# jiaowoguanren0615/Segmentation_Factory

Hardware: AMD Instinct MI355X
Metric: images/sec/GPU fwd+bwd SegFormer-B0 512x512 bf16; mIoU parity vs CPU ref (higher is better)
Workload: dtype bf16; 1 GPU; SegFormer-B0 (MiT-B0 + 768-wide SegFormerHead as the reference builds it), 150 classes, 512x512, full train step (zero_grad+fwd+CE/Dice+bwd+AGC/AdamW); per_gpu_batch=256, global_batch=256, parallelism=dp1, fp8=False, inputs=resident in HBM in the captured step's input buffers (zero-copy feed), launch=hipGraph(zero_grad+fwd+loss+bwd+grad gather) + RCCL all-reduce + fused AGC/AdamW

## Files before the change

### include/segfac.h

```cpp
#ifndef SEGFAC_H
#define SEGFAC_H
#include <stdint.h>

#ifdef __cplusplus
extern "C" {
#endif

#define SEGF_F32 0
#define SEGF_BF16 1
#define SEGF_ERR_SHAPE (-1)
#define SEGF_ERR_DTYPE (-2)
#define SEGF_ERR_WORKSPACE (-3)

const char* segf_version(void);

int segf_cast(const void* src, int src_dt, void* dst, int dst_dt, int64_t n, void* stream);
int segf_cast2d(const void* src, int src_dt, int64_t ld_src, void* dst, int dst_dt, int64_t ld_dst, int64_t rows, int64_t cols,
                void* stream);
int segf_permute021(const void* in, int in_dt, void* out, int out_dt, int64_t A, int64_t Bd, int64_t Cd,
                    int64_t ld_out, void* stream);
typedef struct SegfPrepItem {
    const void* src; void* dst;
    int64_t rows, cols, ld_src, ld_dst, pb, pc;
    int32_t op, src_dt, dst_dt, reserved;
// ... 56 lines not shown
                  const float* pro_shift, int64_t rows_per_group, int act, void* stream);
int segf_bn_affine_table(const float* mean, const float* rstd, const float* gamma, const float* beta, const float* chan_scale,
                         int groups, int C, float* scale, float* shift, void* stream);
int64_t segf_gemm_dw_db_ws(int64_t M, int64_t N, int64_t K, int split_k);
int segf_gemm_dw_db(int dt, int64_t M, int64_t N, int64_t K, const void* A, int64_t lda, const void* B, int64_t ldb,
                    void* C, int c_dt, int64_t ldc, int split_k, float* ws, float* dbias, void* stream);
typedef struct SegfDwItem {
    int64_t M, N, K;
    const void* dy; int64_t lddy;
    const void* x; int64_t ldx;
    float* dw; int64_t lddw;
    float* db;
    float* ws;
    int split_k;
    int shared_split;
} SegfDwItem;
int segf_gemm_dw_db_grouped(int dt, int n, const SegfDwItem* items, void* stream);

int segf_layernorm_fwd(int dt, int64_t rows, int C, const void* x, const float* gamma, const float* beta,
                       float eps, void* y, float* mean, float* rstd, void* stream);
int64_t segf_layernorm_bwd_ws(int64_t rows, int C);
int segf_layernorm_bwd(int dt, int64_t rows, int C, const void* x, const void* dy, const float* gamma,
                       const float* mean, const float* rstd, void* dx, float* dgamma, float* dbeta,
                       float* ws, void* stream);
int segf_layernorm_bwd_fused(int dt, int64_t rows, int C, const void* x, const void* dy, const void* dy2, const void* dres,
                             const float* gamma, const float* mean, const float* rstd, void* dx, float* dgamma, float* dbeta,
                             float* ws, void* stream);
int segf_layernorm_bwd_scaled(int dt, int64_t rows, int C, const void* x, const void* dy, const void* dy2, const void* dres,
                              const float* gamma, const float* mean, const float* rstd, void* dx, float* dgamma, float* dbeta,
                              float* ws, const float* rscale, int64_t rows_per_group, void* dxs, void* stream);
int segf_layernorm_fwd_patch(int dt, int64_t rows, int C, const void* x, const float* gamma, const float* beta, float eps, void* y,
                             float* mean, float* rstd, void* y2, int log2_w, int log2_sr, void* stream);
int segf_layernorm_bwd_patch(int dt, int64_t rows, int C, const void* x, const void* dy, const void* dy2, const void* dres,
                             const float* gamma, const float* mean, const float* rstd, void* dx, float* dgamma, float* dbeta,
                             float* ws, const float* rscale, int64_t rows_per_group, void* dxs, int log2_w, int log2_sr, void* stream);
typedef struct SegfFinalizeItem { const float* partial; float* out; int64_t len; int nblk; int scatter_c; } SegfFinalizeItem;
int segf_layernorm_bwd_blocks(int64_t rows, int C);
int segf_colreduce_finalize_grouped(int n, const SegfFinalizeItem* items, void* stream);
int segf_layernorm_linear_bwd_supported(int dt, int64_t rows, int C, int N);
int segf_layernorm_linear_bwd_blocks(int64_t rows);
int64_t segf_layernorm_linear_bwd_ws(int64_t rows, int C, int N);
int segf_layernorm_linear_bwd(int dt, int64_t rows, int C, int N, const void* dh, const void* w1, const void* x, const void* y,
                              const void* dres, const float* gamma, const float* mean, const float* rstd, void* dx,
                              const float* rscale, int64_t rows_per_group, void* dxs, void* dy_out, float* dw1, float* db1,
                              float* dgamma, float* dbeta, float* ws, void* stream);
int segf_layernorm_linear_bwd_ex_supported(int dt, int64_t rows, int C, int N);
int segf_layernorm_linear_bwd_ex(int dt, int64_t rows, int C, int N, const void* dh, const void* w1, const void* x, const void* y,
                                 const float* beta, const void* dy2, int log2_w, int log2_sr, const void* dres, const float* gamma,
                                 const float* mean, const float* rstd, void* dx, const float* rscale, int64_t rows_per_group, void* dxs,
                                 void* dy_out, float* dw1, float* db1, float* dgamma, float* dbeta, float* ws, void* stream);
int segf_layernorm_linear_fwd_supported(int dt, int64_t rows, int C, int N);
int segf_layernorm_linear_fwd_blocks(int64_t rows);
int segf_layernorm_linear_fwd(int dt, int64_t rows, int C, int N, const void* x, const float* gamma, const float* beta, float eps,
                              const void* w, const float* bias, void* out, float* mean, float* rstd, void* y, void* y2, int log2_w,
                              int log2_sr, void* stream);

int64_t segf_bn_ws(int64_t rows, int C);
int segf_bn_stats(int dt, int64_t rows, int C, const void* x, float* mean, float* rstd,
                  float* running_mean, float* running_var, float momentum, float eps, float* ws, void* stream);
int segf_bn_apply(int dt, int64_t rows, int C, const void* x, const float* mean, const float* rstd,
                  const float* gamma, const float* beta, int act, const float* chan_scale,
                  int64_t rows_per_sample, void* y, void* stream);
int segf_bn_bwd(int dt, int64_t rows, int C, const void* x, const void* dy, const float* mean, const float* rstd,
                const float* gamma, const float* beta, int act, const float* chan_scale, int64_t rows_per_sample,
                int eval_mode, void* dx, float* dgamma, float* dbeta, float* ws, void* stream);

int segf_bn_cls_bwd_supported(int dt, int64_t M, int C, int K, int64_t rows_per_sample);
int64_t segf_bn_cls_bwd_ws(int64_t M, int C, int64_t rows_per_sample);
int segf_bn_cls_bwd(int dt, int64_t M, int C, int K, const void* dy, int64_t ldy, const void* w, int64_t ldw, const void* x,
                    const float* mean, const float* rstd, const float* gamma, const float* beta, int act,
                    const float* chan_scale, int64_t rows_per_sample, int eval_mode, void* dx, float* dgamma, float* dbeta,
                    float* ws, void* stream);
int segf_bn_cls_bwd_dw_supported(int dt, int64_t M, int C, int K, int64_t rows_per_sample, int C1);
int64_t segf_bn_cls_bwd_dw_ws(int64_t M, int C, int64_t rows_per_sample);
int segf_bn_cls_bwd_dw(int dt, int64_t M, int C, int K, const void* dy, int64_t ldy, const void* w, int64_t ldw, const void* x,
                       const float* mean, const float* rstd, const float* gamma, const float* beta, int act,
                       const float* chan_scale, int64_t rows_per_sample, int eval_mode, void* dx, float* dgamma,
                       float* dbeta, float* ws, const void* x1, int64_t ldx1, int C1, float* dG, void* stream);
int64_t segf_bn_cls_bwd_full_ws(int64_t M, int C, int K, int64_t rows_per_sample);
int segf_bn_cls_bwd_full(int dt, int64_t M, int C, int K, const void* dy, int64_t ldy, const void* w, int64_t ldw, const void* x,
                         const float* mean, const float* rstd, const float* gamma, const float* beta, int act,
                         const float* chan_scale, int64_t rows_per_sample, int eval_mode, void* dx, float* dgamma, float* dbeta,
                         float* ws, const void* x1, int64_t ldx1, int C1, float* dG, float* dwcls, void* stream);

int64_t segf_grn_ws(int B, int64_t rows_per_sample, int C, int bwd);
int segf_grn_fwd(int dt, int B, int64_t rows_per_sample, int C, const void* x, const float* gamma, const float* beta, void* y,
                 float* a_scratch, float* sumsq_out, float* ws, int pre_gelu, void* stream);
int segf_grn_bwd(int dt, int B, int64_t rows_per_sample, int C, const void* x, const void* dy, const float* gamma,
                 const float* sumsq_saved, void* dx, float* dgamma, float* dbeta, float* ws, int pre_gelu, void* stream);

int segf_attention_fwd(int dt, int B, int heads, int N, int Nkv, int hd, const void* q, int64_t ldq,
                       const void* k, int64_t ldk, const void* v, int64_t ldv, float scale,
                       void* o, int64_t ldo, float* lse, void* stream);
int64_t segf_attention_bwd_ws(int B, int heads, int N, int Nkv, int hd);
int segf_attention_bwd(int dt, int B, int heads, int N, int Nkv, int hd, const void* q, int64_t ldq,
                       const void* k, int64_t ldk, const void* v, int64_t ldv, float scale,
                       const void* o, int64_t ldo, const void* d_o, int64_t lddo, const float* lse,
                       void* dq, int64_t lddq, void* dk, int64_t lddk, void* dv, int64_t lddv,
                       float* ws, void* stream);

int segf_group_attention_supported(int dt, int B, int H, int W, int heads, int hd, int G, int interval, int lda);
int segf_group_attention_fwd(int dt, int B, int H, int W, int heads, int hd, int G, int interval, int lda, const void* qkv,
                             int64_t ldqkv, const float* bias, float scale, void* o, int64_t ldo, float* lse, void* stream);
int64_t segf_group_attention_bwd_ws(int B, int H, int W, int heads, int hd, int G, int interval, int lda);
int segf_group_attention_bwd(int dt, int B, int H, int W, int heads, int hd, int G, int interval, int lda, const void* qkv,
                             int64_t ldqkv, const float* bias, float scale, const void* d_o, int64_t lddo, const float* lse,
                             void* dqkv, int64_t lddqkv, float* dbias, float* ws, void* stream);

int segf_spatial_gate_supported(int dt, int B, int HW, int C, int64_t ld);
int64_t segf_spatial_gate_fwd_ws(int B, int HW, int C);
int segf_spatial_gate_fwd(int dt, int B, int HW, int C, const void* x, int64_t ldx, const void* r, const float* w, float* s, void* y,
                          int64_t ldy, float* pool, float* ws, void* stream);
int64_t segf_spatial_gate_bwd_ws(int B, int HW, int C);
int segf_spatial_gate_bwd(int dt, int B, int HW, int C, const void* dy, int64_t lddy, const float* dpool, const void* x, int64_t ldx,
                          const void* r, const float* s, const float* w, void* dx, int64_t lddx, void* dr, float* dw, float* ws,
                          void* stream);
int segf_channel_gate_mix_supported(int dt, int B, int HW, int C, int64_t ld);
int segf_channel_gate_mix_fwd(int dt, int B, int HW, int C, const void* q1, int64_t ldq, const void* k1, int64_t ldk, const float* gq,
                              const float* gk, void* u, int64_t ldu, void* stream);
int64_t segf_channel_gate_mix_bwd_ws(int B, int HW, int C);
int segf_channel_gate_mix_bwd(int dt, int B, int HW, int C, const void* du, int64_t lddu, const void* q1, int64_t ldq, const void* k1,
                              int64_t ldk, const float* gq, const float* gk, void* dq1, int64_t lddq, void* dk1, int64_t lddk, float* dgq,
                              float* dgk, float* ws, void* stream);
int segf_gated_mul_supported(int dt, int M, int C, int64_t ld);
int segf_gated_mul_fwd(int dt, int M, int C, const void* a, int64_t lda, const void* v, int64_t ldv, void* z, int64_t ldz, void* stream);
int segf_gated_mul_bwd(int dt, int M, int C, const void* dz, int64_t lddz, const void* a, int64_t lda, const void* v, int64_t ldv,
                       void* da, int64_t ldda, void* dv, int64_t lddv, void* stream);

int segf_starrelu_supported(int dt, int64_t rows, int cols, int64_t ld);
int segf_starrelu_blocks(int64_t rows, int cols);
int segf_starrelu_fwd(int dt, int64_t rows, int cols, const void* u, int64_t ldu, const float* s, const float* b, void* y, int64_t ldy,
                      void* stream);
int64_t segf_starrelu_bwd_ws(int64_t rows, int cols);
int segf_starrelu_bwd(int dt, int64_t rows, int cols, const void* u, int64_t ldu, const void* dy, int64_t lddy, const float* s, void* du,
                      int64_t lddu, float* ds, float* db, float* ws, void* stream);
int segf_colscale_supported(int dt, int64_t rows, int C, int64_t ld);
int segf_colscale_blocks(int64_t rows, int C);
int segf_colscale_fwd(int dt, int64_t rows, int C, const void* x, int64_t ldx, const float* scale, void* y, int64_t ldy, void* stream);
int64_t segf_colscale_bwd_ws(int64_t rows, int C);
int segf_colscale_bwd(int dt, int64_t rows, int C, const void* dy, int64_t lddy, const void* x, int64_t ldx, const float* scale, void* dx,
                      int64_t lddx, float* dscale, float* ws, void* stream);

int segf_dwconv3x3_gelu_fwd(int dt, int B, int H, int W, int C, const void* x, const float* w ,
                            const float* bias, int apply_gelu, void* y, void* stream);
int64_t segf_dwconv3x3_bwd_ws(int B, int H, int W, int C);
int segf_dwconv3x3_bwd_blocks(int dt, int B, int H, int W, int C);
int segf_dwconv3x3_gelu_bwd(int dt, int B, int H, int W, int C, const void* x, const float* w, const float* bias,
                            int apply_gelu, const void* dy, void* du, void* dx, float* dw, float* db,
                            float* ws, void* stream);
int segf_dwconv3x3_gelu_bwd_fc2_supported(int dt, int B, int H, int W, int C_hidden, int C_in);
int segf_dwconv3x3_gelu_bwd_fc2(int dt, int B, int H, int W, int C_hidden, int C_in, const void* f, const float* w9,
                                const float* bias, const void* dys, int64_t ld_dys, const void* w2, void* du, void* dx,
                                float* dw, float* db, float* ws, void* stream);

int segf_dwconv7x7_fwd(int dt, int B, int H, int W, int C, const void* x, const float* wt, const float* bias, void* y,
                       void* stream);
int64_t segf_dwconv7x7_bwd_ws(int B, int H, int W, int C);
int segf_dwconv7x7_bwd(int dt, int B, int H, int W, int C, const void* x, const float* wt, const void* dy, void* dx,
                       float* dw, float* db, float* ws, void* stream);

int segf_conv3x3_fwd_splitk(int mode, int B, int H, int W, int Cin, int Cout);
int segf_conv3x3_pick_splitk(int Cin, int Cout, int64_t P);
int segf_conv3x3(int mode, int B, int H, int W, int Cin, int Cout, const void* x, int64_t ldx, const void* w, int64_t ldw,
                 void* y, int y_dt, int64_t ldy, const float* bias, int split_k, float* ws, void* stream);

int segf_conv3x3_dil_live_taps(int H, int W, int dilation, int* taps );
int segf_conv3x3_dil_supported(int dt, int mode, int B, int H, int W, int Cin, int Cout, int dilation);
int segf_conv3x3_dil_pick_splitk(int B, int H, int W, int Cin, int Cout, int dilation);
int segf_conv3x3_dil(int dt, int mode, int B, int H, int W, int Cin, int Cout, int dilation, const void* x, int64_t ldx,
                     const void* w, int64_t ldw, void* y, int64_t ldy, int split_k, float* ws, void* stream);

int segf_gelu(int dt, int mode, const void* u, const void* dy, void* y, int64_t n, void* stream);
int segf_rowdot(const float* a, int64_t lda, const float* b, int64_t ldb, const float* extra_a, const float* extra_b,
                float* out, int64_t rows, int64_t cols, void* stream);
int segf_adaptive_avgpool(int dt, int bwd, int B, int H, int W, int C, int S, const void* in, void* out, void* stream);

int segf_im2col(int dt, int in_nchw_f32, int B, int H, int W, int Cin, int kh, int kw, int stride, int pad,
                int Ho, int Wo, const void* x, void* col, int64_t ldcol, void* stream);
int segf_col2im(int dt, int B, int H, int W, int Cin, int kh, int kw, int stride, int pad,
                int Ho, int Wo, const void* dcol, int64_t ldcol, void* dx, void* stream);

int segf_bilinear_fwd(int dt, int B, int h, int w, int C, const void* in, int64_t ldi,
                      int H, int W, void* out, int64_t ldo, int align_corners, void* stream);
int segf_bilinear_bwd(int dt, int B, int h, int w, int C, void* din, int64_t ldi,
                      int H, int W, const void* dout, int64_t ldo, int align_corners, void* stream);
int segf_bilinear_bwd_248(int dt, int B, int H, int W, int C, const void* dout, int64_t ldo, void* d2, void* d4, void* d8,
                          void* stream);
int segf_upsample_add(int dt, int B, int H, int W, int C, const void* base, int64_t ldb, int nsrc,
                      const void* src0, int h0, int w0, int64_t ld0, const void* src1, int h1, int w1, int64_t ld1,
                      const void* src2, int h2, int w2, int64_t ld2, void* out, int64_t ldo, int align_corners, void* stream);
int64_t segf_upsample_add_stats_ws(int B, int H, int W, int C);
int segf_upsample_add_stats(int dt, int B, int H, int W, int C, const void* base, int64_t ldb, int nsrc,
                            const void* src0, int h0, int w0, int64_t ld0, const void* src1, int h1, int w1, int64_t ld1,
                            const void* src2, int h2, int w2, int64_t ld2, void* out, int64_t ldo, int align_corners,
                            float* sums, float* ws, void* stream);
int segf_fuse_map_248_supported(int dt, int B, int H, int W, int C, int C1);
int64_t segf_fuse_map_248_ws(int B, int H, int W, int C);
int segf_fuse_map_248(int B, int H, int W, int C, int C1, const void* x1, int64_t ldx1, const void* g1, int64_t ldg,
                      const void* t2, int64_t ld2, const void* t3, int64_t ld3, const void* t4, int64_t ld4,
                      void* out, int64_t ldo, float* sums, float* ws, void* stream);
int segf_bn_stats_from_sums(const float* sums, int64_t rows, int C, float* mean, float* rstd, float* running_mean,
                            float* running_var, float momentum, float eps, void* stream);
int segf_nearest_up(int dt, int bwd, int B, int h, int w, int C, int H, int W, const void* in, const void* base, void* out,
                    void* stream);
int segf_bilinear_to_nchw_f32(int dt, int B, int h, int w, int C, const void* in, int64_t ldi,
                              int H, int W, float* out, void* stream);

int64_t segf_ce_dice_stats_floats(int B, int C);
int64_t segf_ce_dice_lse_floats(int dt, int B, int C, int h, int w, int H, int W, const void* logits, int64_t ldl);
int segf_ce_dice_fwd(int dt, int B, int C, int h, int w, int H, int W, const void* logits, int64_t ldl,
                     const int64_t* target, int64_t ignore_index, const float* class_weight, int dice,
                     float* stats, float* loss, float* pix_lse, void* stream);
int64_t segf_ce_dice_bwd_ws(int dt, int B, int C, int h, int w, int H, int W);
int segf_ce_dice_bwd(int dt, int B, int C, int h, int w, int H, int W, const void* logits, int64_t ldl,
                     const int64_t* target, int64_t ignore_index, const float* class_weight, int dice,
                     const float* stats, const float* grad_out, void* dlogits, int64_t ldd, float* ws,
                     const float* pix_lse, void* stream);

int segf_pixel_loss_supported(int dt, int mode, int B, int C, int h, int w, int H, int W);
int64_t segf_pixel_loss_state_words(int B);
int64_t segf_pixel_loss_bwd_ws(int dt, int B, int C, int h, int w, int H, int W);
int segf_pixel_loss_fwd(int dt, int mode, int B, int C, int h, int w, int H, int W, const void* logits, int64_t ldl,
                        const int64_t* target, int64_t ignore_index, const float* class_weight, float p0, float p1,
                        int size_average, float* ce_map, int32_t* state, float* loss, void* stream);
int segf_pixel_loss_bwd(int dt, int mode, int B, int C, int h, int w, int H, int W, const void* logits, int64_t ldl,
                        const int64_t* target, int64_t ignore_index, const float* class_weight, float p0, float p1,
                        int size_average, const float* ce_map, const int32_t* state, const float* grad_out, void* dlogits,
                        int64_t ldd, float* ws, void* stream);

int segf_debug_wave_reduce16(const float* in, float* out, void* stream);

int segf_argmax_confmat(int dt, int B, int C, int h, int w, int H, int W, const void* logits, int64_t ldl,
                        const int64_t* target, int64_t ignore_label, int64_t* mat, int64_t* hist,
                        int32_t* flag, int64_t* pred_out , void* stream);

#define SEGF_MSF_MAX_MAPS 16
// ... 83 lines not shown
```

### segmentation_factory_amd/csrc/conv.hip

```cpp
#include <stdlib.h>
#include "colreduce.h"

#define DW_PIX 4

template <typename T, int MODE>
__global__ void __launch_bounds__(256) dwconv3x3_kernel(const T* __restrict__ x, const float* __restrict__ w,
                                                         const float* __restrict__ bias, int apply_gelu,
                                                         const T* __restrict__ dy, T* __restrict__ y, int B, int H, int W, int C) {
    const int nchunk = C / 8;
    const int wg = (W + DW_PIX - 1) / DW_PIX;
    const int units = B * H * wg;
    const int64_t g = (int64_t)xcd_block() * 256 + threadIdx.x;
    const int ustep = (int)(((int64_t)gridDim.x * 256) / nchunk);
    const int c0 = (int)(g % nchunk) * 8;
    f32x2_t wk[9][4], bs[4];
#pragma unroll
    for (int jj = 0; jj < 4; ++jj) {
#pragma unroll
        for (int kk = 0; kk < 9; ++kk) {
            const int ks = MODE == 1 ? 8 - kk : kk;
            wk[kk][jj] = f32x2_t{w[(c0 + 2 * jj) * 9 + ks], w[(c0 + 2 * jj + 1) * 9 + ks]};
        }
        bs[jj] = (MODE != 1 && bias) ? f32x2_t{bias[c0 + 2 * jj], bias[c0 + 2 * jj + 1]} : f32x2_t{0.f, 0.f};
    }
// ... 149 lines not shown
        if (MODE == 2) { load_grow(ya - 2, grawb[0]); load_grow(ya - 1, grawb[1]); }
        int yin = ya - 1;
        for (int st = 0; st < steps; ++st) {
#pragma unroll
            for (int j = 0; j < 3; ++j, ++yin) {
                f32x2_t (&P)[DW_PIX][2] = acc[j % 3];
                f32x2_t (&Cc)[DW_PIX][2] = acc[(j + 1) % 3];
                f32x2_t (&N)[DW_PIX][2] = acc[(j + 2) % 3];
                Raw4<T> (&curc)[DW_PIX + 2] = rawb[j % 3];
                Raw4<T> (&gcurc)[DW_PIX] = grawb[j % 3];
                load_row(yin + 2, rawb[(j + 2) % 3]);
                if (MODE == 2) load_grow(yin + 1, grawb[(j + 2) % 3]);
                const bool vy = yin >= 0 && yin < H && yin <= yb;
#pragma unroll
                for (int cx = 0; cx < DW_PIX + 2; ++cx) {
                    f32x2_t v[2];
                    unpack4v(curc[cx], vy && cok[cx], v);
#pragma unroll
                    for (int kx = 0; kx < 3; ++kx) {
                        const int p = cx - kx;
                        if (p >= 0 && p < DW_PIX) {
#pragma unroll
                            for (int jj = 0; jj < 2; ++jj) {
                                P[p][jj] = wk[6 + kx][jj] * v[jj] + P[p][jj];
                                Cc[p][jj] = wk[3 + kx][jj] * v[jj] + Cc[p][jj];
                                N[p][jj] = wk[kx][jj] * v[jj] + N[p][jj];
                            }
                        }
                    }
                }
                const int yo = yin - 1;
                if (yo >= ya && yo < yb) {
                    T* orow = yo_b + (int64_t)yo * W * C;
#pragma unroll
                    for (int h = 0; h < DW_PIX / 2; ++h) {
                        f32x2_t a8[4] = {P[2 * h][0], P[2 * h][1], P[2 * h + 1][0], P[2 * h + 1][1]};
                        if (MODE == 0 && apply_gelu) gelu_erf8<false>(a8, nullptr);
                        if (MODE == 2) {
                            f32x2_t gy[4], g0[2], g1[2];
                            unpack4v(gcurc[2 * h], true, g0); unpack4v(gcurc[2 * h + 1], true, g1);
                            gy[0] = g0[0]; gy[1] = g0[1]; gy[2] = g1[0]; gy[3] = g1[1];
                            if (apply_gelu) gelu_erf8<true>(a8, gy);
                            else { a8[0] = gy[0]; a8[1] = gy[1]; a8[2] = gy[2]; a8[3] = gy[3]; }
                        }
                        const f32x2_t o0[2] = {a8[0], a8[1]}, o1[2] = {a8[2], a8[3]};
                        if (cok[2 * h + 1]) store4v(orow + coff[2 * h + 1], o0);
                        if (cok[2 * h + 2]) store4v(orow + coff[2 * h + 2], o1);
                    }
                }
#pragma unroll
                for (int p = 0; p < DW_PIX; ++p) { P[p][0] = bs[0]; P[p][1] = bs[1]; }
            }
        }
    }
}

static inline void dw_walk_plan(int H, int& R, int& nseg, int64_t columns = 0) {
    nseg = (H + 63) / 64;
    while (columns > 0 && columns * nseg < 131072 && (H + nseg - 1) / nseg > 8) nseg *= 2;
    if (POL(dw_walk_rows) > 0) nseg = (H + POL(dw_walk_rows) - 1) / POL(dw_walk_rows);
    R = (H + nseg - 1) / nseg;
}
static inline bool dw_use_walk() { return !POL(dw_no_walk); }
template <typename T, int MODE>
static inline void dw_walk_launch(hipStream_t st, const T* x, const float* w, const float* bias, int apply_gelu, const T* dy, T* y,
                                  int B, int H, int W, int C) {
    int R, nseg;
    dw_walk_plan(H, R, nseg, (int64_t)B * ((W + DW_PIX - 1) / DW_PIX) * (C / 4));
    const int64_t units = (int64_t)B * nseg * ((W + DW_PIX - 1) / DW_PIX);
    const int blocks = colfixed_blocks(units, C / 4, 1, 32768);
    hipLaunchKernelGGL((dwconv3x3_walk_kernel<T, MODE>), dim3(blocks), dim3(256), 0, st, x, w, bias, apply_gelu, dy, y, B, H, W, C, R, nseg);
}

typedef __attribute__((ext_vector_type(8))) __bf16 dwf_bf16x8;
typedef __attribute__((ext_vector_type(4))) float dwf_f32x4;
typedef __attribute__((ext_vector_type(8))) short dwf_s16x8;
typedef uint32_t dwf_u32x4 __attribute__((ext_vector_type(4)));
template <int KS>
__global__ void __launch_bounds__(256, 2) dwconv3x3_walk_fc2_kernel(const bf16_t* __restrict__ x, const float* __restrict__ w,
                                                                     const float* __restrict__ bias, const bf16_t* __restrict__ dys,
                                                                     int64_t ld_dys, const bf16_t* __restrict__ w2,
                                                                     bf16_t* __restrict__ y, int B, int H, int W, int C, int R, int nseg) {
    typedef bf16_t T;
    const int lane = threadIdx.x & 63;
    const int n = lane & 15, g = lane >> 4;
    const int nslab = C / 64;
    const int nrun = (W + 15) / 16;
    const int units = B * nseg * nrun;
    const int wv = __builtin_amdgcn_readfirstlane((int)(xcd_block() * 4 + (threadIdx.x >> 6)));
    const int ustep = (int)((gridDim.x * 4) / nslab);
    const int cbase = (wv % nslab) * 64;
    const int c0 = cbase + 4 * n;
    f32x2_t wk[9][2], bs[2];
#pragma unroll
    for (int jj = 0; jj < 2; ++jj) {
#pragma unroll
        for (int kk = 0; kk < 9; ++kk) wk[kk][jj] = f32x2_t{w[(c0 + 2 * jj) * 9 + kk], w[(c0 + 2 * jj + 1) * 9 + kk]};
        bs[jj] = bias ? f32x2_t{bias[c0 + 2 * jj], bias[c0 + 2 * jj + 1]} : f32x2_t{0.f, 0.f};
    }
    dwf_bf16x8 Bf[4][KS];
#pragma unroll
    for (int s = 0; s < KS; ++s) {
        dwf_s16x8 t[4];
#pragma unroll
        for (int e = 0; e < 8; ++e) {
            const uint2 q = *reinterpret_cast<const uint2*>(w2 + (int64_t)(32 * s + 8 * g + e) * C + c0);
            t[0][e] = (short)(q.x & 0xffffu); t[1][e] = (short)(q.x >> 16); t[2][e] = (short)(q.y & 0xffffu); t[3][e] = (short)(q.y >> 16);
        }
#pragma unroll
        for (int j = 0; j < 4; ++j) Bf[j][s] = __builtin_bit_cast(dwf_bf16x8, t[j]);
    }
    const int steps = (R + 2 + 2) / 3;
    for (int u = wv / nslab; u < units; u += ustep) {
        const int run = u % nrun;
        const int t = u / nrun;
        const int seg = t % nseg;
        const int b = t / nseg;
        const int x0 = run * 16 + 4 * g;
        const int ya = seg * R, yb = ya + R < H ? ya + R : H;
        const T* xb = x + (int64_t)b * H * W * C + c0;
        T* yo_b = y + (int64_t)b * H * W * C + c0;
        const int tpx = run * 16 + n < W ? run * 16 + n : W - 1;
        const T* gb = dys + ((int64_t)b * H * W + tpx) * ld_dys + 8 * g;
        int coff[DW_PIX + 2];
        bool cok[DW_PIX + 2];
#pragma unroll
        for (int cx = 0; cx < DW_PIX + 2; ++cx) {
            const int ix = x0 + cx - 1;
            cok[cx] = ix >= 0 && ix < W;
            coff[cx] = (ix < 0 ? 0 : (ix >= W ? W - 1 : ix)) * C;
        }
        f32x2_t acc[3][DW_PIX][2];
#pragma unroll
        for (int a = 0; a < 3; ++a)
#pragma unroll
            for (int p = 0; p < DW_PIX; ++p) { acc[a][p][0] = bs[0]; acc[a][p][1] = bs[1]; }
        Raw4<T> rawb[3][DW_PIX + 2];
        dwf_u32x4 dysb[3][KS];
        auto load_row = [&](int yin, Raw4<T> (&dst)[DW_PIX + 2]) {
            const int yc = yin < 0 ? 0 : (yin >= H ? H - 1 : yin);
            const T* row = xb + (int64_t)yc * W * C;
#pragma unroll
            for (int cx = 0; cx < DW_PIX + 2; ++cx) dst[cx] = load4_raw<T>(row + coff[cx]);
        };
        auto load_grow = [&](int yo, dwf_u32x4 (&dst)[KS]) {
            const int yc = yo < 0 ? 0 : (yo >= H ? H - 1 : yo);
            const T* row = gb + (int64_t)yc * W * ld_dys;
#pragma unroll
            for (int s = 0; s < KS; ++s) dst[s] = *reinterpret_cast<const dwf_u32x4*>(row + 32 * s);
        };
        load_row(ya - 1, rawb[0]);
        load_row(ya, rawb[1]);
        load_grow(ya - 2, dysb[0]); load_grow(ya - 1, dysb[1]);
        int yin = ya - 1;
        for (int st = 0; st < steps; ++st) {
#pragma unroll
            for (int j = 0; j < 3; ++j, ++yin) {
                f32x2_t (&P)[DW_PIX][2] = acc[j % 3];
                f32x2_t (&Cc)[DW_PIX][2] = acc[(j + 1) % 3];
                f32x2_t (&N)[DW_PIX][2] = acc[(j + 2) % 3];
                Raw4<T> (&curc)[DW_PIX + 2] = rawb[j % 3];
                dwf_u32x4 (&gcurc)[KS] = dysb[j % 3];
                load_row(yin + 2, rawb[(j + 2) % 3]);
                load_grow(yin + 1, dysb[(j + 2) % 3]);
                const bool vy = yin >= 0 && yin < H && yin <= yb;
#pragma unroll
                for (int cx = 0; cx < DW_PIX + 2; ++cx) {
                    f32x2_t v[2];
                    unpack4v(curc[cx], vy && cok[cx], v);
#pragma unroll
                    for (int kx = 0; kx < 3; ++kx) {
                        const int p = cx - kx;
                        if (p >= 0 && p < DW_PIX) {
#pragma unroll
                            for (int jj = 0; jj < 2; ++jj) {
                                P[p][jj] = wk[6 + kx][jj] * v[jj] + P[p][jj];
                                Cc[p][jj] = wk[3 + kx][jj] * v[jj] + Cc[p][jj];
                                N[p][jj] = wk[kx][jj] * v[jj] + N[p][jj];
                            }
                        }
                    }
                }
                const int yo = yin - 1;
                if (yo >= ya && yo < yb) {
                    dwf_f32x4 dgf[4];
#pragma unroll
                    for (int jm = 0; jm < 4; ++jm) {
                        dgf[jm] = dwf_f32x4{0.f, 0.f, 0.f, 0.f};
#pragma unroll
                        for (int s = 0; s < KS; ++s)
                            dgf[jm] = __builtin_amdgcn_mfma_f32_16x16x32_bf16(__builtin_bit_cast(dwf_bf16x8, gcurc[s]), Bf[jm][s], dgf[jm], 0, 0, 0);
                    }
                    T* orow = yo_b + (int64_t)yo * W * C;
#pragma unroll
                    for (int h = 0; h < DW_PIX / 2; ++h) {
                        f32x2_t a8[4] = {P[2 * h][0], P[2 * h][1], P[2 * h + 1][0], P[2 * h + 1][1]};
                        Raw4<T> q0, q1;
                        q0.u.x = pack2bf(dgf[0][2 * h], dgf[1][2 * h]); q0.u.y = pack2bf(dgf[2][2 * h], dgf[3][2 * h]);
                        q1.u.x = pack2bf(dgf[0][2 * h + 1], dgf[1][2 * h + 1]); q1.u.y = pack2bf(dgf[2][2 * h + 1], dgf[3][2 * h + 1]);
                        f32x2_t gy[4], g0[2], g1[2];
                        unpack4v(q0, true, g0); unpack4v(q1, true, g1);
                        gy[0] = g0[0]; gy[1] = g0[1]; gy[2] = g1[0]; gy[3] = g1[1];
                        gelu_erf8<true>(a8, gy);
                        const f32x2_t o0[2] = {a8[0], a8[1]}, o1[2] = {a8[2], a8[3]};
                        if (cok[2 * h + 1]) store4v(orow + coff[2 * h + 1], o0);
                        if (cok[2 * h + 2]) store4v(orow + coff[2 * h + 2], o1);
                    }
                }
#pragma unroll
                for (int p = 0; p < DW_PIX; ++p) { P[p][0] = bs[0]; P[p][1] = bs[1]; }
            }
        }
    }
}

static inline int dw_blocks(int B, int H, int W, int C) {
    return colfixed_blocks((int64_t)B * H * ((W + DW_PIX - 1) / DW_PIX), C / 8, 8, 16384);
}

extern "C" int segf_dwconv3x3_gelu_fwd(int dt, int B, int H, int W, int C, const void* x, const float* w, const float* bias,
                                       int apply_gelu, void* y, void* stream) {
    if (B <= 0 || H <= 0 || W <= 0) return 0;
    if (C <= 0 || C % 8 != 0 || ((uintptr_t)x % 16) || ((uintptr_t)y % 16)) return SEGF_ERR_SHAPE;
    if ((int64_t)B * H * W >= (1ll << 31)) return SEGF_ERR_SHAPE;
    hipStream_t st = (hipStream_t)stream;
    const int blocks = dw_blocks(B, H, W, C);
    SEGF_DISPATCH_DT(dt, T, {
        if (dw_use_walk()) dw_walk_launch<T, 0>(st, (const T*)x, w, bias, apply_gelu, (const T*)nullptr, (T*)y, B, H, W, C);
        else
        hipLaunchKernelGGL((dwconv3x3_kernel<T, 0>), dim3(blocks), dim3(256), 0, st, (const T*)x, w, bias, apply_gelu,
                           (const T*)nullptr, (T*)y, B, H, W, C);
    })
    SEGF_CHECK_LAUNCH();
    return 0;
}

#define DWG_MAX_BLOCKS 1024
struct DwgPlan { int ch, rl, slabs, nblk, units_per_blk; };
static inline DwgPlan dwg_plan(int B, int H, int W, int C) {
    DwgPlan p;
    const int nchunk = C / 8;
    p.ch = nchunk < 256 ? nchunk : 256;
    p.rl = 256 / p.ch;
    p.slabs = (nchunk + p.ch - 1) / p.ch;
    const int64_t units = (int64_t)B * H * ((W + DW_PIX - 1) / DW_PIX);
    int64_t want = cdiv64(units, (int64_t)p.rl * 4);
    int cap = DWG_MAX_BLOCKS / p.slabs;
    if (cap < 1) cap = 1;
    p.nblk = (int)(want < 1 ? 1 : (want > cap ? cap : want));
    p.units_per_blk = (int)cdiv64(units, p.nblk);
    return p;
}

template <typename T>
__global__ void __launch_bounds__(256) dwconv3x3_wgrad_kernel(const T* __restrict__ x, const T* __restrict__ du,
                                                               float* __restrict__ partial, int B, int H, int W, int C, int ch,
                                                               int rl, int units_per_blk) {
    __shared__ float red[256 * 8];
    const int tx = threadIdx.x % ch, ty = threadIdx.x / ch;
    const int chunk = blockIdx.y * ch + tx;
    const int c0 = chunk * 8;
    const bool active = ty < rl && c0 < C;
    const int wg = (W + DW_PIX - 1) / DW_PIX;
    const int units = B * H * wg;
    float acc[10][8];
#pragma unroll
    for (int o = 0; o < 10; ++o)
#pragma unroll
        for (int j = 0; j < 8; ++j) acc[o][j] = 0.f;
    (void)units_per_blk;
    if (active) {
        for (int u = (int)xcd_block() * rl + ty; u < units; u += (int)gridDim.x * rl) {
            const int xg = u % wg;
            const int t = u / wg;
// ... 316 lines not shown
static inline int dw_small_nch(int dt, int B, int H, int W, int C) {
    if (POL(dw_no_small) || C % 8 || B > 4096) return 0;
    const int HW = H * W, umax = dt == SEGF_BF16 ? 1024 : 512;
    if (HW > umax || HW < 16) return 0;
    for (int nch = 4; nch >= 1; nch >>= 1)
        if (HW * nch <= umax && (C / 8) % nch == 0) {
            if ((int64_t)B * (C / (8 * nch)) > 512 && !POL(dw_small_always)) return 0;
            return nch;
        }
    return 0;
}

extern "C" int64_t segf_dwconv3x3_bwd_ws(int B, int H, int W, int C) {
    DwgPlan p = dwg_plan(B, H, W, C > 0 ? C : 8);
    DwwPlan q = dww_plan(B, H > 0 ? H : 1, W > 0 ? W : 1, C > 0 ? C : 8);
    int nblk = p.nblk > q.nblk ? p.nblk : q.nblk;
    if (B > nblk) nblk = B;
    return (int64_t)nblk * 10 * C + 10 * (int64_t)C;
}

extern "C" int segf_dwconv3x3_gelu_bwd(int dt, int B, int H, int W, int C, const void* x, const float* w, const float* bias,
                                       int apply_gelu, const void* dy, void* du, void* dx, float* dw, float* db, float* ws,
                                       void* stream) {
    if (B <= 0 || H <= 0 || W <= 0) return 0;
    if (C <= 0 || C % 8 != 0 || ((uintptr_t)x % 16) || ((uintptr_t)dy % 16) || ((uintptr_t)du % 16) || ((uintptr_t)dx % 16))
        return SEGF_ERR_SHAPE;
    if ((int64_t)B * H * W >= (1ll << 31)) return SEGF_ERR_SHAPE;
    if (!ws) return SEGF_ERR_WORKSPACE;
    hipStream_t st = (hipStream_t)stream;
    if (const int nch = dw_small_nch(dt, B, H, W, C)) {
        const size_t esz = dt == SEGF_BF16 ? 2 : 4;
        const size_t shm = (size_t)H * W * nch * 8 * esz * 2 + (size_t)nch * 80 * 4 + 256 * 8 * 4;
        const int blocks = B * (C / (8 * nch));
        SEGF_DISPATCH_DT(dt, T, {
            hipLaunchKernelGGL((dwconv3x3_bwd_small_kernel<T>), dim3(blocks), dim3(256), shm, st, (const T*)x, w, bias, apply_gelu,
                               (const T*)dy, (T*)dx, ws, B, H, W, C, nch);
        })
        SEGF_CHECK_LAUNCH();
        if (!dw) return 0;
        float* sums_s = ws + (int64_t)B * 10 * C;
        colreduce_finalize_launch(ws, B, 10 * (int64_t)C, sums_s, st);
        SEGF_CHECK_LAUNCH();
        hipLaunchKernelGGL(dw_scatter_kernel, dim3((C + 255) / 256), dim3(256), 0, st, sums_s, C, dw, db);
        SEGF_CHECK_LAUNCH();
        return 0;
    }
    DwgPlan p = dwg_plan(B, H, W, C);
    const DwwPlan q = dww_plan(B, H, W, C);
    const bool walk = dw_use_walk();
    if (walk) p.nblk = q.nblk;
    float* sums = ws + (int64_t)p.nblk * 10 * C;
    const int blocks = dw_blocks(B, H, W, C);
    SEGF_DISPATCH_DT(dt, T, {
        if (dw_use_walk()) dw_walk_launch<T, 2>(st, (const T*)x, w, bias, apply_gelu, (const T*)dy, (T*)du, B, H, W, C);
        else
        hipLaunchKernelGGL((dwconv3x3_kernel<T, 2>), dim3(blocks), dim3(256), 0, st, (const T*)x, w, bias, apply_gelu,
                           (const T*)dy, (T*)du, B, H, W, C);
        if (walk)
        hipLaunchKernelGGL((dwconv3x3_wgrad_walk_kernel<T>), dim3(q.nblk, q.slabs), dim3(256), 0, st, (const T*)x, (const T*)du, ws,
                           B, H, W, C, q.ch, q.rl, q.R, q.nseg);
        else
        hipLaunchKernelGGL((dwconv3x3_wgrad_kernel<T>), dim3(p.nblk, p.slabs), dim3(256), 0, st, (const T*)x, (const T*)du, ws,
                           B, H, W, C, p.ch, p.rl, p.units_per_blk);
        if (dw_use_walk()) dw_walk_launch<T, 1>(st, (const T*)du, w, (const float*)nullptr, 0, (const T*)nullptr, (T*)dx, B, H, W, C);
        else
        hipLaunchKernelGGL((dwconv3x3_kernel<T, 1>), dim3(blocks), dim3(256), 0, st, (const T*)du, w, (const float*)nullptr, 0,
                           (const T*)nullptr, (T*)dx, B, H, W, C);
    })
    SEGF_CHECK_LAUNCH();
    if (!dw) return 0;
    colreduce_finalize_launch(ws, p.nblk, 10 * (int64_t)C, sums, st);
    SEGF_CHECK_LAUNCH();
    hipLaunchKernelGGL(dw_scatter_kernel, dim3((C + 255) / 256), dim3(256), 0, st, sums, C, dw, db);
    SEGF_CHECK_LAUNCH();
    return 0;
}
extern "C" int segf_dwconv3x3_bwd_blocks(int dt, int B, int H, int W, int C) {
    if (B <= 0 || H <= 0 || W <= 0 || C <= 0) return 0;
    if (dw_small_nch(dt, B, H, W, C)) return B;
    return dw_use_walk() ? dww_plan(B, H, W, C).nblk : dwg_plan(B, H, W, C).nblk;
}

#define DW_FC2_MIN_ROWS 131072
static inline bool dw_fc2_shape_ok(int dt, int B, int H, int W, int C, int Cin) {
    return dt == SEGF_BF16 && B > 0 && H > 0 && W > 0 && (Cin == 32 || Cin == 64) && C > 0 && C % 64 == 0 &&
           (int64_t)B * H * W < (1ll << 31);
}
extern "C" int segf_dwconv3x3_gelu_bwd_fc2_supported(int dt, int B, int H, int W, int C_hidden, int C_in) {
    if (!dw_fc2_shape_ok(dt, B, H, W, C_hidden, C_in)) return 0;
    if (!dw_use_walk() || dw_small_nch(dt, B, H, W, C_hidden)) return 0;
    const int pol = POL(ffn_bwd_fused);
    if (pol <= 0) return 0;
    if (pol >= 2) return 1;
    return (int64_t)B * H * W >= DW_FC2_MIN_ROWS;
}
extern "C" int segf_dwconv3x3_gelu_bwd_fc2(int dt, int B, int H, int W, int C_hidden, int C_in, const void* f, const float* w9,
                                           const float* bias, const void* dys, int64_t ld_dys, const void* w2, void* du, void* dx,
                                           float* dw, float* db, float* ws, void* stream) {
    if (B <= 0 || H <= 0 || W <= 0) return 0;
    const int C = C_hidden;
    if (dt != SEGF_BF16) return SEGF_ERR_DTYPE;
    if (!dw_fc2_shape_ok(dt, B, H, W, C, C_in) || !dw_use_walk() || dw_small_nch(dt, B, H, W, C)) return SEGF_ERR_SHAPE;
    if (((uintptr_t)f % 16) || ((uintptr_t)dys % 16) || ((uintptr_t)w2 % 16) || ((uintptr_t)du % 16) || ((uintptr_t)dx % 16) ||
        ld_dys < C_in || ld_dys % 8 != 0)
        return SEGF_ERR_SHAPE;
    if (!ws) return SEGF_ERR_WORKSPACE;
    hipStream_t st = (hipStream_t)stream;
    typedef bf16_t T;
    const DwwPlan q = dww_plan(B, H, W, C);
    float* sums = ws + (int64_t)q.nblk * 10 * C;
    {
        const int nslab = C / 64;
        const int64_t waves = (int64_t)B * q.nseg * ((W + 15) / 16) * nslab;
        int64_t blocks = (waves + 3) / 4;
        if (blocks > 32768) blocks = 32768;
        blocks = (blocks + nslab - 1) / nslab * nslab;
        if (C_in == 32)
            hipLaunchKernelGGL((dwconv3x3_walk_fc2_kernel<1>), dim3((unsigned)blocks), dim3(256), 0, st, (const T*)f, w9, bias, (const T*)dys,
                               ld_dys, (const T*)w2, (T*)du, B, H, W, C, q.R, q.nseg);
        else
            hipLaunchKernelGGL((dwconv3x3_walk_fc2_kernel<2>), dim3((unsigned)blocks), dim3(256), 0, st, (const T*)f, w9, bias, (const T*)dys,
                               ld_dys, (const T*)w2, (T*)du, B, H, W, C, q.R, q.nseg);
    }
    hipLaunchKernelGGL((dwconv3x3_wgrad_walk_kernel<T>), dim3(q.nblk, q.slabs), dim3(256), 0, st, (const T*)f, (const T*)du, ws,
                       B, H, W, C, q.ch, q.rl, q.R, q.nseg);
    dw_walk_launch<T, 1>(st, (const T*)du, w9, (const float*)nullptr, 0, (const T*)nullptr, (T*)dx, B, H, W, C);
    SEGF_CHECK_LAUNCH();
    if (!dw) return 0;
    colreduce_finalize_launch(ws, q.nblk, 10 * (int64_t)C, sums, st);
    SEGF_CHECK_LAUNCH();
    hipLaunchKernelGGL(dw_scatter_kernel, dim3((C + 255) / 256), dim3(256), 0, st, sums, C, dw, db);
    SEGF_CHECK_LAUNCH();
    return 0;
}

#define DW7_PIX 8
template <typename T, bool FLIP>
__global__ void __launch_bounds__(256) dwconv7x7_kernel(const T* __restrict__ x, const float* __restrict__ wt,
                                                         const float* __restrict__ bias, T* __restrict__ y, int B, int H, int W, int C) {
    const int nchunk = C / 8;
    const int wg = (W + DW7_PIX - 1) / DW7_PIX;
    const int units = B * H * wg;
    const int64_t g = (int64_t)xcd_block() * 256 + threadIdx.x;
    const int ustep = (int)(((int64_t)gridDim.x * 256) / nchunk);
    const int c0 = (int)(g % nchunk) * 8;
    f32x2_t bs[4];
#pragma unroll
    for (int jj = 0; jj < 4; ++jj) bs[jj] = (!FLIP && bias) ? f32x2_t{bias[c0 + 2 * jj], bias[c0 + 2 * jj + 1]} : f32x2_t{0.f, 0.f};
    for (int u = (int)(g / nchunk); u < units; u += ustep) {
        const int xg = u % wg;
        const int t = u / wg;
        const int yy = t % H;
        const int b = t / H;
        const int x0 = xg * DW7_PIX;
        f32x2_t acc[DW7_PIX][4];
#pragma unroll
        for (int p = 0; p < DW7_PIX; ++p)
#pragma unroll
            for (int jj = 0; jj < 4; ++jj) acc[p][jj] = bs[jj];
        for (int ky = 0; ky < 7; ++ky) {
            const int iy = yy + ky - 3;
            if (iy < 0 || iy >= H) continue;
            f32x2_t wk[7][4];
#pragma unroll
            for (int kx = 0; kx < 7; ++kx) {
                const float* wp = wt + (int64_t)(FLIP ? 48 - (ky * 7 + kx) : ky * 7 + kx) * C + c0;
                const float4 wa = *reinterpret_cast<const float4*>(wp), wb = *reinterpret_cast<const float4*>(wp + 4);
                wk[kx][0] = f32x2_t{wa.x, wa.y}; wk[kx][1] = f32x2_t{wa.z, wa.w};
                wk[kx][2] = f32x2_t{wb.x, wb.y}; wk[kx][3] = f32x2_t{wb.z, wb.w};
            }
            const T* row = x + (((int64_t)b * H + iy) * W) * C + c0;
#pragma unroll
            for (int half = 0; half < 2; ++half) {
                Raw8<T> raw[7];
#pragma unroll
                for (int q = 0; q < 7; ++q) {
                    const int ix = x0 + half * 7 + q - 3;
                    raw[q] = load8_raw<T>(row + (int64_t)(ix < 0 ? 0 : (ix >= W ? W - 1 : ix)) * C);
                }
                SEGF_LOADS_ISSUED();
#pragma unroll
                for (int q = 0; q < 7; ++q) {
                    const int cx = half * 7 + q;
                    const int ix = x0 + cx - 3;
                    f32x2_t v[4];
                    zero_unless(raw[q], ix >= 0 && ix < W);
                    unpack8v<T>(raw[q], v);
#pragma unroll
                    for (int kx = 0; kx < 7; ++kx) {
                        const int p = cx - kx;
                        if (p >= 0 && p < DW7_PIX) {
#pragma unroll
                            for (int jj = 0; jj < 4; ++jj) acc[p][jj] = wk[kx][jj] * v[jj] + acc[p][jj];
                        }
                    }
                }
            }
        }
#pragma unroll
        for (int p = 0; p < DW7_PIX; ++p)
// ... 450 lines not shown
```

### segmentation_factory_amd/csrc/elementwise.hip

```cpp
#include "colreduce.h"

extern "C" const char* segf_version(void) { return "segfac-hip 0.1 gfx950"; }

template <typename S, typename D>
__global__ void cast_kernel(const S* __restrict__ src, D* __restrict__ dst, int64_t n, bool vec) {
    const int64_t stride = (int64_t)gridDim.x * blockDim.x;
    if (vec) {
        const int64_t n8 = n / 8;
        for (int64_t i = (int64_t)blockIdx.x * blockDim.x + threadIdx.x; i < n8; i += stride) {
            float v[8];
            load8<S>(src + i * 8, v);
            store8<D>(dst + i * 8, v);
        }
        for (int64_t i = n8 * 8 + (int64_t)blockIdx.x * blockDim.x + threadIdx.x; i < n; i += stride)
            stf<D>(dst + i, ldf<S>(src + i));
    } else {
        for (int64_t i = (int64_t)blockIdx.x * blockDim.x + threadIdx.x; i < n; i += stride)
            stf<D>(dst + i, ldf<S>(src + i));
    }
}

extern "C" int segf_cast(const void* src, int src_dt, void* dst, int dst_dt, int64_t n, void* stream) {
    if (n <= 0) return 0;
    hipStream_t st = (hipStream_t)stream;
// ... 303 lines not shown
}
extern "C" int segf_event_destroy(void* event) { return (int)hipEventDestroy((hipEvent_t)event); }
extern "C" int segf_event_record(void* event, void* stream, int external) {
    hipStream_t st = (hipStream_t)stream;
    hipEvent_t ev = (hipEvent_t)event;
    if (!external) return (int)hipEventRecord(ev, st);
    hipStreamCaptureStatus status = hipStreamCaptureStatusNone;
    hipGraph_t graph = nullptr;
    const hipGraphNode_t* deps = nullptr;
    size_t ndeps = 0;
    hipError_t r = hipStreamGetCaptureInfo_v2(st, &status, nullptr, &graph, &deps, &ndeps);
    if (r != hipSuccess) return (int)r;
    if (status != hipStreamCaptureStatusActive) return SEGF_ERR_SHAPE;
    r = hipEventRecordWithFlags(ev, st, hipEventRecordExternal);
    if (r == hipSuccess) return 0;
    (void)hipGetLastError();
    hipGraphNode_t node = nullptr;
    r = hipGraphAddEventRecordNode(&node, graph, deps, ndeps, ev);
    if (r != hipSuccess) return (int)r;
    r = hipStreamUpdateCaptureDependencies(st, &node, 1, hipStreamSetCaptureDependencies);
    return (int)r;
}
extern "C" int segf_stream_wait_event(void* stream, void* event) {
    return (int)hipStreamWaitEvent((hipStream_t)stream, (hipEvent_t)event, 0);
}


__global__ void zero_fill_kernel(uint32_t* __restrict__ p, int64_t nwords, uint8_t* __restrict__ tail, int ntail) {
    for (int64_t i = (int64_t)blockIdx.x * blockDim.x + threadIdx.x; i < nwords; i += (int64_t)gridDim.x * blockDim.x) p[i] = 0u;
    if (blockIdx.x == 0 && (int)threadIdx.x < ntail) tail[threadIdx.x] = 0;
}
extern "C" int segf_zero(void* p, int64_t nbytes, void* stream) {
    if (nbytes <= 0) return 0;
    if ((uintptr_t)p % 4) return SEGF_ERR_SHAPE;
    const int64_t nwords = nbytes / 4;
    const int blocks = (int)imin64(cdiv64(nwords > 0 ? nwords : 1, 256), 4096);
    hipLaunchKernelGGL(zero_fill_kernel, dim3(blocks), dim3(256), 0, (hipStream_t)stream, (uint32_t*)p, nwords,
                       (uint8_t*)p + nwords * 4, (int)(nbytes - nwords * 4));
    SEGF_CHECK_LAUNCH();
    return 0;
}
__global__ void hist_accum_kernel(float* __restrict__ hist, int64_t* __restrict__ counts, int64_t n, int clear) {
    const int64_t i = (int64_t)blockIdx.x * blockDim.x + threadIdx.x;
    if (i >= n) return;
    hist[i] += (float)counts[i];
    if (clear) counts[i] = 0;
}
extern "C" int segf_hist_accum(float* hist, int64_t* counts, int64_t n, int clear, void* stream) {
    if (n <= 0) return 0;
    if (!hist || !counts) return SEGF_ERR_SHAPE;
    hipLaunchKernelGGL(hist_accum_kernel, dim3((unsigned)cdiv64(n, 256)), dim3(256), 0, (hipStream_t)stream, hist, counts, n, clear);
    SEGF_CHECK_LAUNCH();
    return 0;
}
__global__ void debug_spin_kernel(int64_t ticks) {
    const uint64_t t0 = __builtin_amdgcn_s_memrealtime();
    for (int guard = 0; guard < (1 << 24); ++guard) {
        if ((int64_t)(__builtin_amdgcn_s_memrealtime() - t0) >= ticks) break;
        __builtin_amdgcn_s_sleep(32);
    }
}
extern "C" int segf_debug_spin(int64_t us, void* stream) {
    if (us < 0 || us > 200000) return SEGF_ERR_SHAPE;
    hipLaunchKernelGGL(debug_spin_kernel, dim3(1), dim3(64), 0, (hipStream_t)stream, us * 100);
    SEGF_CHECK_LAUNCH();
    return 0;
}
__global__ void add_i64_kernel(int64_t* p, int64_t v) { if (threadIdx.x == 0) *p += v; }
extern "C" int segf_add_i64(int64_t* p, int64_t v, void* stream) {
    hipLaunchKernelGGL(add_i64_kernel, dim3(1), dim3(64), 0, (hipStream_t)stream, p, v);
    SEGF_CHECK_LAUNCH();
    return 0;
}

__device__ __forceinline__ uint64_t splitmix64(uint64_t z) {
    z += 0x9E3779B97F4A7C15ull;
    z = (z ^ (z >> 30)) * 0xBF58476D1CE4E5B9ull;
    z = (z ^ (z >> 27)) * 0x94D049BB133111EBull;
    return z ^ (z >> 31);
}
__global__ void bernoulli_scale_kernel(uint64_t* __restrict__ state, const float* __restrict__ kp, int64_t n, int64_t row_len,
                                       float* __restrict__ out) {
    const uint64_t seed = state[0], ctr = state[1];
    for (int64_t i = (int64_t)blockIdx.x * blockDim.x + threadIdx.x; i < n; i += (int64_t)gridDim.x * blockDim.x) {
        const uint64_t r = splitmix64(splitmix64(seed ^ (ctr * 0xD1B54A32D192ED03ull)) + (uint64_t)i);
        const float u = (float)(r >> 40) * (1.f / 16777216.f);
        const float k = kp[i / row_len];
        out[i] = u < k ? 1.f / k : 0.f;
    }
    __syncthreads();
    if (gridDim.x == 1 && threadIdx.x == 0) state[1] = ctr + 1;
}
extern "C" int segf_bernoulli_scale(uint64_t* state, const float* keep_prob, int64_t n, int64_t row_len, float* out, void* stream) {
    if (n <= 0) return 0;
    if (row_len <= 0 || n > (1 << 20)) return SEGF_ERR_SHAPE;
    hipLaunchKernelGGL(bernoulli_scale_kernel, dim3(1), dim3(1024), 0, (hipStream_t)stream, state, keep_prob, n, row_len, out);
    SEGF_CHECK_LAUNCH();
    return 0;
}
```

### segmentation_factory_amd/csrc/head_fused.hip

```cpp
#include "colreduce.h"

typedef __attribute__((ext_vector_type(8))) __bf16 hf_bf16x8;
typedef __attribute__((ext_vector_type(4))) float hf_f32x4;
typedef __attribute__((ext_vector_type(8))) short hf_s16x8;

struct HeadFusedArgs {
    const bf16_t* dy; int64_t ldy;
    const bf16_t* w; int64_t ldw;
    const bf16_t* x;
    const float *mean, *rstd, *gamma, *beta;
    const float* cscale;
    const float* sums;
    bf16_t* dx;
    float* partial;
    int64_t M; int C; int64_t rps; int groups_per_sample, chunks_per_sample; int act, eval_mode;
    const bf16_t* x1; int64_t ldx1;
    float* dwpart;
    float* cwpart;
};
#define DW_C1 32
#define DW_LD 40

__device__ __forceinline__ hf_bf16x8 hf_frag_tok_tr(const unsigned char* tile, int rowbytes, int cb, int lane) {
    typedef __attribute__((ext_vector_type(4))) short hf_s16x4;
    const int g = lane >> 4, i = lane & 15, q = i >> 2, p = i & 3;
    const unsigned char* a0 = tile + (8 * g + q) * rowbytes + (cb + 4 * p) * 2;
    const hf_s16x4 lo = __builtin_amdgcn_ds_read_tr16_b64_v4i16((__attribute__((address_space(3))) hf_s16x4*)a0);
    const hf_s16x4 hi = __builtin_amdgcn_ds_read_tr16_b64_v4i16((__attribute__((address_space(3))) hf_s16x4*)(a0 + 4 * rowbytes));
    const hf_s16x8 v = __builtin_shufflevector(lo, hi, 0, 1, 2, 3, 4, 5, 6, 7);
    return __builtin_bit_cast(hf_bf16x8, v);
}

__device__ __forceinline__ float hf_row_sum16(float v) {
    v += dpp_mov<DPP_XOR1>(v); v += dpp_mov<DPP_XOR2>(v); v += dpp_mov<DPP_HALF_MIRROR>(v); v += dpp_mov<DPP_MIRROR>(v);
    return v;
}

#ifndef HF_WAVES
#define HF_WAVES 8
#endif
#ifndef HF_OCC
#define HF_OCC 1
#endif
#ifndef HF_U
#define HF_U 4
#endif
template <int PASS, int KS, bool DW = false, bool CW = false>
__global__ void __launch_bounds__(64 * HF_WAVES, HF_OCC) bn_cls_bwd_kernel(HeadFusedArgs a) {
    constexpr int NT = 2;
    constexpr int TOK = 16 * HF_U;
    constexpr int RS = 32 * KS + 8;
    constexpr int NCH = TOK * 4 * KS;
    constexpr int CPT = (NCH + 64 * HF_WAVES - 1) / (64 * HF_WAVES);
    __shared__ __attribute__((aligned(16))) bf16_t tile[2][TOK][RS];
    constexpr int XW = 32 * HF_WAVES;
    constexpr int XRS = XW + 8;
    constexpr int XCH = TOK * (XW / 8);
    constexpr int XPT = XCH / (64 * HF_WAVES);
    static_assert(XCH % (64 * HF_WAVES) == 0, "x tile chunks must divide evenly over the workgroup");
    __shared__ __attribute__((aligned(16))) bf16_t xt[2][TOK][XRS];
    __shared__ __attribute__((aligned(16))) bf16_t ot[PASS == 2 ? TOK : 1][XRS];
    static_assert(!DW || (PASS == 2 && HF_WAVES == 8 && TOK == 64), "the riding weight gradient belongs to pass 2");
    static_assert(!CW || (PASS == 1 && TOK % 32 == 0), "the classifier's weight gradient rides on pass 1");
    __shared__ __attribute__((aligned(16))) bf16_t at[CW ? TOK : 1][XRS];
    hf_f32x4 accc[CW ? 2 * KS : 1][CW ? 2 : 1];
#pragma unroll
    for (int i = 0; i < (CW ? 2 * KS : 1); ++i)
#pragma unroll
        for (int j = 0; j < (CW ? 2 : 1); ++j) accc[i][j] = hf_f32x4{0.f, 0.f, 0.f, 0.f};
    constexpr int X1RS = DW_C1 + 16 + 8;
    __shared__ __attribute__((aligned(16))) bf16_t x1t[DW ? 2 : 1][DW ? TOK : 1][X1RS];
    const int lane = threadIdx.x & 63, wave = threadIdx.x >> 6;
    const int mi = lane & 15, g = lane >> 4;
    const unsigned L = xcd_block();
    const int ny = a.C / (32 * HF_WAVES);
    const int slice = (int)(L % (unsigned)ny), blk = (int)(L / (unsigned)ny);
    const int n0 = (slice * HF_WAVES + wave) * (16 * NT);
    hf_bf16x8 Wf[NT][KS];
#pragma unroll
    for (int nt = 0; nt < NT; ++nt) {
        const int n = n0 + 8 * (mi >> 2) + 4 * nt + (mi & 3);
#pragma unroll
        for (int s = 0; s < KS; ++s) {
            hf_s16x8 wv;
#pragma unroll
            for (int j = 0; j < 8; ++j) wv[j] = (short)a.w[(int64_t)(32 * s + 8 * g + j) * a.ldw + n];
            Wf[nt][s] = __builtin_bit_cast(hf_bf16x8, wv);
        }
    }
    const int f0 = n0 + 8 * g;
    float zA[8], zB[8], hC[8], hD[8], E[8], P[8], Q[8];
    const float invn = 1.f / (float)a.M;
#pragma unroll
    for (int j = 0; j < 8; ++j) {
        const float mu = a.mean[f0 + j], rs = a.rstd[f0 + j], ga = a.gamma[f0 + j], be = a.beta[f0 + j];
        zA[j] = ga * rs; zB[j] = be - mu * ga * rs;
        hC[j] = rs; hD[j] = -mu * rs;
        if (PASS == 2) {
            const float mg = a.eval_mode ? 0.f : a.sums[f0 + j] * invn, mgx = a.eval_mode ? 0.f : a.sums[a.C + f0 + j] * invn;
            E[j] = ga * rs;
            P[j] = ga * rs * (mg + hD[j] * mgx);
            Q[j] = ga * rs * hC[j] * mgx;
        }
    }
    const float zlo = a.act == 0 ? -INFINITY : 0.f, zhi = a.act == 2 ? 6.f : INFINITY;
    float s1[8], s2[8];
#pragma unroll
    for (int j = 0; j < 8; ++j) { s1[j] = 0.f; s2[j] = 0.f; }
    const int b = blk / a.chunks_per_sample, chunk = blk % a.chunks_per_sample;
    const int gbeg = (int)((int64_t)a.groups_per_sample * chunk / a.chunks_per_sample);
    const int gend = (int)((int64_t)a.groups_per_sample * (chunk + 1) / a.chunks_per_sample);
    float cs[8];
#pragma unroll
    for (int j = 0; j < 8; ++j) {
        cs[j] = a.cscale ? a.cscale[(int64_t)b * a.C + f0 + j] : 1.f;
        if (PASS == 2) E[j] *= cs[j];
        if (CW) { zA[j] *= cs[j]; zB[j] *= cs[j]; }
    }
    const int64_t row0 = (int64_t)b * a.rps;
    const int64_t last_row = row0 + (int64_t)gend * 16 - 1;
    static_assert(CPT <= 3, "dy tile: at most three 16-byte chunks per thread");
    uint4 stg0 = make_uint4(0, 0, 0, 0), stg1 = make_uint4(0, 0, 0, 0), stg2 = make_uint4(0, 0, 0, 0);
    auto fetch_one = [&](int gp, int q) -> uint4 {
        q = q < NCH ? q : NCH - 1;
        const int tk = q / (4 * KS), col = q % (4 * KS);
        int64_t m = row0 + (int64_t)gp * 16 + tk;
        m = m <= last_row ? m : last_row;
        return *reinterpret_cast<const uint4*>(a.dy + m * a.ldy + 8 * col);
    };
    auto fetch_tile = [&](int gp) {
        stg0 = fetch_one(gp, (int)threadIdx.x);
        if (CPT > 1) stg1 = fetch_one(gp, (int)threadIdx.x + 64 * HF_WAVES);
        if (CPT > 2) stg2 = fetch_one(gp, (int)threadIdx.x + 128 * HF_WAVES);
    };
    auto stash_one = [&](int bufi, int q, const uint4& v) {
        const int tk = q / (4 * KS), col = q % (4 * KS);
        if (q < NCH) *reinterpret_cast<uint4*>(&tile[bufi][tk][8 * col]) = v;
    };
    auto stash_tile = [&](int bufi) {
        stash_one(bufi, (int)threadIdx.x, stg0);
        if (CPT > 1) stash_one(bufi, (int)threadIdx.x + 64 * HF_WAVES, stg1);
        if (CPT > 2) stash_one(bufi, (int)threadIdx.x + 128 * HF_WAVES, stg2);
    };
    typedef uint32_t hf_u32x4 __attribute__((ext_vector_type(4)));
    hf_u32x4 xs[XPT];
    const int wg_f0 = slice * XW;
    auto fetch_x = [&](int gp) {
#pragma unroll
        for (int i = 0; i < XPT; ++i) {
            const int q = (int)threadIdx.x + 64 * HF_WAVES * i, tk = q / (XW / 8), c16 = q % (XW / 8);
            int64_t m = row0 + (int64_t)gp * 16 + tk;
            m = m <= last_row ? m : last_row;
            xs[i] = *reinterpret_cast<const hf_u32x4*>(a.x + m * a.C + wg_f0 + 8 * c16);
        }
    };
    auto stash_x = [&](int bufi) {
#pragma unroll
        for (int i = 0; i < XPT; ++i) {
            const int q = (int)threadIdx.x + 64 * HF_WAVES * i, tk = q / (XW / 8), c16 = q % (XW / 8);
            *reinterpret_cast<hf_u32x4*>(&xt[bufi][tk][8 * c16]) = xs[i];
        }
    };
    hf_u32x4 x1s = {0u, 0u, 0u, 0u};
    auto fetch_x1 = [&](int gp) {
        if (DW) {
            const int q = (int)threadIdx.x & 255, tk = q >> 2, c16 = q & 3;
            int64_t m = row0 + (int64_t)gp * 16 + tk;
            m = m <= last_row ? m : last_row;
            x1s = *reinterpret_cast<const hf_u32x4*>(a.x1 + m * a.ldx1 + 8 * c16);
        }
    };
    auto stash_x1 = [&](int bufi, int gp) {
        if (DW) {
            const int t = (int)threadIdx.x;
            if (t < 256) {
                const int tk = t >> 2, c16 = t & 3;
                const bool live = gp + (tk >> 4) < gend;
                const hf_u32x4 z = {0u, 0u, 0u, 0u};
                *reinterpret_cast<hf_u32x4*>(&x1t[bufi][tk][8 * c16]) = live ? x1s : z;
            } else if (t < 384) {
                const int r = t - 256, tk = r >> 1, half = r & 1;
                const bool live = gp + (tk >> 4) < gend;
                const hf_u32x4 v = {(half == 0 && live) ? 0x00003f80u : 0u, 0u, 0u, 0u};
                *reinterpret_cast<hf_u32x4*>(&x1t[bufi][tk][DW_C1 + 8 * half]) = v;
            }
        }
    };
    hf_f32x4 accw[DW ? 2 : 1][DW ? 3 : 1];
#pragma unroll
    for (int i = 0; i < (DW ? 2 : 1); ++i)
#pragma unroll
        for (int j = 0; j < (DW ? 3 : 1); ++j) accw[i][j] = hf_f32x4{0.f, 0.f, 0.f, 0.f};
    if (gbeg < gend) { fetch_tile(gbeg); fetch_x(gbeg); fetch_x1(gbeg); stash_tile(0); stash_x(0); stash_x1(0, gbeg); }
    __syncthreads();
    int bufi = 0;
    for (int gp = gbeg; gp < gend; gp += HF_U) {
        const bool more = gp + HF_U < gend;
        if (more) { fetch_tile(gp + HF_U); fetch_x(gp + HF_U); fetch_x1(gp + HF_U); }
        constexpr int UNR = CW ? 1 : HF_U;
#pragma unroll UNR
        for (int u = 0; u < HF_U; ++u) {
            hf_f32x4 acc[NT];
#pragma unroll
            for (int nt = 0; nt < NT; ++nt) acc[nt] = hf_f32x4{0.f, 0.f, 0.f, 0.f};
#pragma unroll
            for (int s = 0; s < KS; ++s) {
                const hf_bf16x8 yv = *reinterpret_cast<const hf_bf16x8*>(&tile[bufi][16 * u + mi][32 * s + 8 * g]);
#pragma unroll
                for (int nt = 0; nt < NT; ++nt) acc[nt] = __builtin_amdgcn_mfma_f32_16x16x32_bf16(Wf[nt][s], yv, acc[nt], 0, 0, 0);
            }
            const bool live = gp + u < gend;
            const hf_u32x4 xv4 = *reinterpret_cast<const hf_u32x4*>(&xt[bufi][16 * u + mi][32 * wave + 8 * g]);
            const uint32_t xw[4] = {xv4[0], xv4[1], xv4[2], xv4[3]};
            float o[8];
#pragma unroll
            for (int j = 0; j < 8; ++j) {
                const float da = j < 4 ? acc[0][j] : acc[1][j - 4];
                const float xv = (j & 1) ? __uint_as_float(xw[j >> 1] & 0xffff0000u) : __uint_as_float(xw[j >> 1] << 16);
                const float z = fmaf(xv, zA[j], zB[j]);
                const bool on = live & (z > zlo) & (z < zhi);
                const float gm = on ? da : 0.f;
                if (PASS == 1) {
                    s1[j] += gm;
                    s2[j] = fmaf(gm, xv, s2[j]);
                    if (CW) o[j] = live ? fmaxf(z, zlo) : 0.f;
                } else {
                    o[j] = fmaf(E[j], gm, -fmaf(xv, Q[j], P[j]));
                }
            }
            if (CW) {
                const hf_u32x4 av = {pack2bf(o[0], o[1]), pack2bf(o[2], o[3]), pack2bf(o[4], o[5]), pack2bf(o[6], o[7])};
                *reinterpret_cast<hf_u32x4*>(&at[16 * u + mi][32 * wave + 8 * g]) = av;
            }
            if (PASS == 2) {
                const hf_u32x4 ov = {pack2bf(o[0], o[1]), pack2bf(o[2], o[3]), pack2bf(o[4], o[5]), pack2bf(o[6], o[7])};
                *reinterpret_cast<hf_u32x4*>(&ot[16 * u + mi][32 * wave + 8 * g]) = ov;
            }
        }
        if (CW) {
            __builtin_amdgcn_fence(__ATOMIC_ACQ_REL, "wavefront");
            __builtin_amdgcn_wave_barrier();
#pragma unroll
            for (int ks = 0; ks < TOK / 32; ++ks) {
                const unsigned char* ab = reinterpret_cast<const unsigned char*>(&at[32 * ks][0]);
                const unsigned char* yb = reinterpret_cast<const unsigned char*>(&tile[bufi][32 * ks][0]);
                const hf_bf16x8 fb0 = hf_frag_tok_tr(ab, XRS * 2, 32 * wave, lane), fb1 = hf_frag_tok_tr(ab, XRS * 2, 32 * wave + 16, lane);
#pragma unroll
                for (int ct = 0; ct < 2 * KS; ++ct) {
                    const hf_bf16x8 fa = hf_frag_tok_tr(yb, RS * 2, 16 * ct, lane);
                    accc[ct][0] = __builtin_amdgcn_mfma_f32_16x16x32_bf16(fa, fb0, accc[ct][0], 0, 0, 0);
                    accc[ct][1] = __builtin_amdgcn_mfma_f32_16x16x32_bf16(fa, fb1, accc[ct][1], 0, 0, 0);
                    if (ct & 1) __builtin_amdgcn_sched_barrier(0);
                }
            }
            __builtin_amdgcn_fence(__ATOMIC_ACQ_REL, "wavefront");
            __builtin_amdgcn_wave_barrier();
        }
        __builtin_amdgcn_sched_barrier(0);
        asm volatile("" ::: "memory");
        if (more) {
            stash_tile(bufi ^ 1);
            stash_x(bufi ^ 1);
            stash_x1(bufi ^ 1, gp + HF_U);
        }
        __syncthreads();
        if (DW) {
#pragma unroll
            for (int ks = 0; ks < TOK / 32; ++ks) {
                const unsigned char* ob = reinterpret_cast<const unsigned char*>(&ot[32 * ks][0]);
                const unsigned char* xb = reinterpret_cast<const unsigned char*>(&x1t[bufi][32 * ks][0]);
                const hf_bf16x8 fa0 = hf_frag_tok_tr(ob, XRS * 2, 32 * wave, lane), fa1 = hf_frag_tok_tr(ob, XRS * 2, 32 * wave + 16, lane);
#pragma unroll
                for (int nt = 0; nt < 3; ++nt) {
                    const hf_bf16x8 fb = hf_frag_tok_tr(xb, X1RS * 2, 16 * nt, lane);
                    accw[0][nt] = __builtin_amdgcn_mfma_f32_16x16x32_bf16(fa0, fb, accw[0][nt], 0, 0, 0);
                    accw[1][nt] = __builtin_amdgcn_mfma_f32_16x16x32_bf16(fa1, fb, accw[1][nt], 0, 0, 0);
                }
            }
        }
        if (PASS == 2) {
#pragma unroll
            for (int i = 0; i < XPT; ++i) {
                const int q = (int)threadIdx.x + 64 * HF_WAVES * i, tk = q / (XW / 8), c16 = q % (XW / 8);
                const hf_u32x4 ov = *reinterpret_cast<const hf_u32x4*>(&ot[tk][8 * c16]);
                if (gp + (tk >> 4) < gend)
                    *reinterpret_cast<hf_u32x4*>(a.dx + (row0 + (int64_t)gp * 16 + tk) * a.C + wg_f0 + 8 * c16) = ov;
            }
            __syncthreads();
        }
        bufi ^= 1;
    }
    if (DW) {
        float* dst = a.dwpart + ((int64_t)blk * a.C + wg_f0 + 32 * wave) * DW_LD;
#pragma unroll
        for (int mt = 0; mt < 2; ++mt)
#pragma unroll
            for (int nt = 0; nt < 3; ++nt) {
                const int cc = 16 * nt + mi;
                if (cc < DW_LD) {
#pragma unroll
                    for (int r = 0; r < 4; ++r) dst[(16 * mt + 4 * g + r) * DW_LD + cc] = accw[mt][nt][r];
                }
            }
    }
    if (CW) {
        float* dst = a.cwpart + (int64_t)blk * (32 * KS) * a.C + wg_f0 + 32 * wave + mi;
#pragma unroll
        for (int ct = 0; ct < 2 * KS; ++ct)
#pragma unroll
            for (int ft = 0; ft < 2; ++ft)
#pragma unroll
                for (int r = 0; r < 4; ++r) dst[(int64_t)(16 * ct + 4 * g + r) * a.C + 16 * ft] = accc[ct][ft][r];
    }
    if (PASS == 1) {
        float* dst = a.partial + (int64_t)blk * 2 * a.C + f0;
#pragma unroll
        for (int j = 0; j < 8; ++j) {
            const float r1 = hf_row_sum16(s1[j]), r2 = hf_row_sum16(s2[j]);
            const float csj = a.cscale ? a.cscale[(int64_t)b * a.C + f0 + j] : 1.f;
            const float hCj = a.rstd[f0 + j], hDj = -a.mean[f0 + j] * hCj;
            if (mi == 0) { dst[j] = csj * r1; dst[a.C + j] = csj * fmaf(hCj, r2, hDj * r1); }
        }
    }
}

__global__ void hf_split_kernel(const float* __restrict__ sums, int C, float* __restrict__ dgamma, float* __restrict__ dbeta) {
    const int c = blockIdx.x * blockDim.x + threadIdx.x;
    if (c >= C) return;
    dbeta[c] = sums[c];
    dgamma[c] = sums[C + c];
}

static int hf_chunks(int B, int groups_per_sample, int ny, bool cw = false) {
    const int budget = cw ? 768 : 3072;
    int s = (budget / ny + B - 1) / B;
    if (s > groups_per_sample / 8) s = groups_per_sample / 8;
    return s < 1 ? 1 : s;
}

extern "C" int segf_bn_cls_bwd_supported(int dt, int64_t M, int C, int K, int64_t rows_per_sample) {
    if (dt != SEGF_BF16 || POL(no_head_fused)) return 0;
    if (K % 32 || K < 32 || K > 192 || C % (32 * HF_WAVES) || rows_per_sample <= 0 || rows_per_sample % 16 || M % rows_per_sample) return 0;
    if (M / rows_per_sample > 65535 || M < 16384) return 0;
    return 1;
}
extern "C" int64_t segf_bn_cls_bwd_ws(int64_t M, int C, int64_t rows_per_sample) {
    const int B = (int)(M / rows_per_sample);
    return (int64_t)B * hf_chunks(B, (int)(rows_per_sample / 16), C / (32 * HF_WAVES)) * 2 * C + 2 * C;
}

extern "C" int64_t segf_bn_cls_bwd_full_ws(int64_t M, int C, int K, int64_t rows_per_sample) {
    const int B = (int)(M / rows_per_sample);
    const int gps = (int)(rows_per_sample / 16), ny = C / (32 * HF_WAVES);
    const int64_t nb_cw = (int64_t)B * hf_chunks(B, gps, ny, true), nb_plain = (int64_t)B * hf_chunks(B, gps, ny, false);
    const int64_t nblk = nb_cw > nb_plain ? nb_cw : nb_plain;
    return nblk * 2 * C + 2 * C + nblk * C * DW_LD + nb_cw * (int64_t)K * C;
}

extern "C" int segf_bn_cls_bwd_dw_supported(int dt, int64_t M, int C, int K, int64_t rows_per_sample, int C1) {
    if (POL(no_head_fused_dw)) return 0;
    return segf_bn_cls_bwd_supported(dt, M, C, K, rows_per_sample) && C1 == DW_C1 && K <= 160;
}
extern "C" int64_t segf_bn_cls_bwd_dw_ws(int64_t M, int C, int64_t rows_per_sample) {
    const int B = (int)(M / rows_per_sample);
    return segf_bn_cls_bwd_ws(M, C, rows_per_sample) +
           (int64_t)B * hf_chunks(B, (int)(rows_per_sample / 16), C / (32 * HF_WAVES)) * C * DW_LD;
}

static int bn_cls_bwd_impl(int dt, int64_t M, int C, int K, const void* dy, int64_t ldy, const void* w, int64_t ldw, const void* x,
                           const float* mean, const float* rstd, const float* gamma, const float* beta, int act,
                           const float* chan_scale, int64_t rows_per_sample, int eval_mode, void* dx, float* dgamma,
                           float* dbeta, float* ws, const void* x1, int64_t ldx1, float* dG, void* stream, float* dwcls = nullptr);

extern "C" int segf_bn_cls_bwd_full(int dt, int64_t M, int C, int K, const void* dy, int64_t ldy, const void* w, int64_t ldw,
                                    const void* x, const float* mean, const float* rstd, const float* gamma, const float* beta, int act,
                                    const float* chan_scale, int64_t rows_per_sample, int eval_mode, void* dx, float* dgamma,
                                    float* dbeta, float* ws, const void* x1, int64_t ldx1, int C1, float* dG, float* dwcls,
                                    void* stream) {
    if (x1 && (!segf_bn_cls_bwd_dw_supported(dt, M, C, K, rows_per_sample, C1) || !dG || ldx1 < C1 || ldx1 % 8 || ((uintptr_t)x1 % 16)))
        return SEGF_ERR_SHAPE;
    if (dwcls && (K > 192 || act > 1)) return SEGF_ERR_SHAPE;
    return bn_cls_bwd_impl(dt, M, C, K, dy, ldy, w, ldw, x, mean, rstd, gamma, beta, act, chan_scale, rows_per_sample, eval_mode, dx,
                           dgamma, dbeta, ws, x1, ldx1, x1 ? dG : nullptr, stream, dwcls);
}

extern "C" int segf_bn_cls_bwd(int dt, int64_t M, int C, int K, const void* dy, int64_t ldy, const void* w, int64_t ldw, const void* x,
                               const float* mean, const float* rstd, const float* gamma, const float* beta, int act,
                               const float* chan_scale, int64_t rows_per_sample, int eval_mode, void* dx, float* dgamma,
                               float* dbeta, float* ws, void* stream) {
    return bn_cls_bwd_impl(dt, M, C, K, dy, ldy, w, ldw, x, mean, rstd, gamma, beta, act, chan_scale, rows_per_sample, eval_mode, dx,
                           dgamma, dbeta, ws, nullptr, 0, nullptr, stream);
}
extern "C" int segf_bn_cls_bwd_dw(int dt, int64_t M, int C, int K, const void* dy, int64_t ldy, const void* w, int64_t ldw, const void* x,
                                  const float* mean, const float* rstd, const float* gamma, const float* beta, int act,
                                  const float* chan_scale, int64_t rows_per_sample, int eval_mode, void* dx, float* dgamma,
                                  float* dbeta, float* ws, const void* x1, int64_t ldx1, int C1, float* dG, void* stream) {
    if (!segf_bn_cls_bwd_dw_supported(dt, M, C, K, rows_per_sample, C1) || !x1 || !dG || ldx1 < C1 || ldx1 % 8 || ((uintptr_t)x1 % 16))
        return SEGF_ERR_SHAPE;
    return bn_cls_bwd_impl(dt, M, C, K, dy, ldy, w, ldw, x, mean, rstd, gamma, beta, act, chan_scale, rows_per_sample, eval_mode, dx,
                           dgamma, dbeta, ws, x1, ldx1, dG, stream);
}

static int bn_cls_bwd_impl(int dt, int64_t M, int C, int K, const void* dy, int64_t ldy, const void* w, int64_t ldw, const void* x,
                           const float* mean, const float* rstd, const float* gamma, const float* beta, int act,
                           const float* chan_scale, int64_t rows_per_sample, int eval_mode, void* dx, float* dgamma,
                           float* dbeta, float* ws, const void* x1, int64_t ldx1, float* dG, void* stream, float* dwcls) {
    if (!segf_bn_cls_bwd_supported(dt, M, C, K, rows_per_sample) || ldy < K || ldw < C || act < 0 || act > 2) return SEGF_ERR_SHAPE;
    if (((uintptr_t)dy | (uintptr_t)x | (uintptr_t)dx) % 16 || (ldy % 8)) return SEGF_ERR_SHAPE;
    if (!ws) return SEGF_ERR_WORKSPACE;
    hipStream_t st = (hipStream_t)stream;
    const int B = (int)(M / rows_per_sample), gps = (int)(rows_per_sample / 16), ny = C / (32 * HF_WAVES);
    const int chunks = hf_chunks(B, gps, ny, dwcls != nullptr);
    const int nblk = B * chunks;
    float* sums = ws + (int64_t)nblk * 2 * C;
    float* dwpart = sums + 2 * C;
    float* cwpart = dwpart + (int64_t)nblk * C * DW_LD;
    HeadFusedArgs a{(const bf16_t*)dy, ldy, (const bf16_t*)w, ldw, (const bf16_t*)x, mean, rstd, gamma, beta, chan_scale, sums,
                    (bf16_t*)dx, ws, M, C, rows_per_sample, gps, chunks, act, eval_mode, (const bf16_t*)x1, ldx1, dwpart, cwpart};
    const dim3 grid((unsigned)(nblk * ny));
#define HF_LAUNCH(PASS)                                                                                                  \
    do {                                                                                                                 \
        switch (K / 32) {                                                                                                \
        case 1: hipLaunchKernelGGL((bn_cls_bwd_kernel<PASS, 1>), grid, dim3(64 * HF_WAVES), 0, st, a); break;                      \
        case 2: hipLaunchKernelGGL((bn_cls_bwd_kernel<PASS, 2>), grid, dim3(64 * HF_WAVES), 0, st, a); break;                      \
        case 3: hipLaunchKernelGGL((bn_cls_bwd_kernel<PASS, 3>), grid, dim3(64 * HF_WAVES), 0, st, a); break;                      \
        case 4: hipLaunchKernelGGL((bn_cls_bwd_kernel<PASS, 4>), grid, dim3(64 * HF_WAVES), 0, st, a); break;                      \
        case 5: hipLaunchKernelGGL((bn_cls_bwd_kernel<PASS, 5>), grid, dim3(64 * HF_WAVES), 0, st, a); break;                      \
        default: hipLaunchKernelGGL((bn_cls_bwd_kernel<PASS, 6>), grid, dim3(64 * HF_WAVES), 0, st, a); break;                     \
        }                                                                                                                \
    } while (0)
    if (dwcls) {
        switch (K / 32) {
        case 1: hipLaunchKernelGGL((bn_cls_bwd_kernel<1, 1, false, true>), grid, dim3(64 * HF_WAVES), 0, st, a); break;
        case 2: hipLaunchKernelGGL((bn_cls_bwd_kernel<1, 2, false, true>), grid, dim3(64 * HF_WAVES), 0, st, a); break;
        case 3: hipLaunchKernelGGL((bn_cls_bwd_kernel<1, 3, false, true>), grid, dim3(64 * HF_WAVES), 0, st, a); break;
        case 4: hipLaunchKernelGGL((bn_cls_bwd_kernel<1, 4, false, true>), grid, dim3(64 * HF_WAVES), 0, st, a); break;
        case 5: hipLaunchKernelGGL((bn_cls_bwd_kernel<1, 5, false, true>), grid, dim3(64 * HF_WAVES), 0, st, a); break;
        default: hipLaunchKernelGGL((bn_cls_bwd_kernel<1, 6, false, true>), grid, dim3(64 * HF_WAVES), 0, st, a); break;
        }
        SEGF_CHECK_LAUNCH();
        colreduce_finalize_launch(cwpart, nblk, (int64_t)K * C, dwcls, st);
    } else {
        HF_LAUNCH(1);
    }
    SEGF_CHECK_LAUNCH();
    colreduce_finalize_launch(ws, nblk, 2 * (int64_t)C, sums, st);
    SEGF_CHECK_LAUNCH();
    if (x1) {
        switch (K / 32) {
        case 1: hipLaunchKernelGGL((bn_cls_bwd_kernel<2, 1, true>), grid, dim3(64 * HF_WAVES), 0, st, a); break;
        case 2: hipLaunchKernelGGL((bn_cls_bwd_kernel<2, 2, true>), grid, dim3(64 * HF_WAVES), 0, st, a); break;
        case 3: hipLaunchKernelGGL((bn_cls_bwd_kernel<2, 3, true>), grid, dim3(64 * HF_WAVES), 0, st, a); break;
        case 4: hipLaunchKernelGGL((bn_cls_bwd_kernel<2, 4, true>), grid, dim3(64 * HF_WAVES), 0, st, a); break;
        default: hipLaunchKernelGGL((bn_cls_bwd_kernel<2, 5, true>), grid, dim3(64 * HF_WAVES), 0, st, a); break;
        }
        SEGF_CHECK_LAUNCH();
        colreduce_finalize_launch(dwpart, nblk, (int64_t)C * DW_LD, dG, st);
    } else {
        HF_LAUNCH(2);
    }
    SEGF_CHECK_LAUNCH();
#undef HF_LAUNCH
    hipLaunchKernelGGL(hf_split_kernel, dim3((C + 255) / 256), dim3(256), 0, st, sums, C, dgamma, dbeta);
    SEGF_CHECK_LAUNCH();
    return 0;
}
```

### segmentation_factory_amd/csrc/loss.hip

```cpp
#include <stdlib.h>
#include "colreduce.h"

#include "loss_geom.h"

static inline int pow2_scale(int h, int w, int H, int W) {
    if (h <= 0 || w <= 0 || H % h || W % w) return 0;
    const int sc = H / h;
    if (W / w != sc || (sc & (sc - 1)) || sc > 8) return 0;
    return sc;
}

template <typename T, int NS>
__device__ __forceinline__ void load_tap(const T* __restrict__ p, int lane, int C, float (&t)[NS]) {
#pragma unroll
    for (int s = 0; s < NS; ++s) {
        const int c = lane + 64 * s;
        const float v = ldf<T>(p + (c < C ? c : C - 1));
        t[s] = c < C ? v : 0.f;
    }
}

template <typename T, int NS, bool ATEN = false>
__device__ __forceinline__ void pixel_logits(const T* __restrict__ img, const LossGeom& g, int Y, int X, int lane, float (&z)[NS]) {
    if (g.h == g.H && g.w == g.W) {
// ... 288 lines not shown
#pragma unroll
    for (int s = 0; s < NS; ++s) { aI[s] = 0.f; aP[s] = 0.f; aT[s] = 0.f; }
    float ce = 0.f, wsum = 0.f, nvalid = 0.f, bad = 0.f;
    for (int cell = blockIdx.x * 4 + wave; cell < ncell; cell += gridDim.x * 4) {
        const Cell c = make_cell(cell / ncx - halo, cell % ncx - halo, g.h, g.w, halo);
        float t00[NS], t01[NS], t10[NS], t11[NS];
        load_cell_taps<T, NS>(img, g, c, lane, t00, t01, t10, t11);
        const int codes = cell_label_codes(tg, g, sc, off, c.cj, c.ck, lane, ignore_index);
        const float mb = cell_max_bound<NS>(t00, t01, t10, t11, lane, g.C);
        for (int a = 0; a < sc; ++a) {
            const int Y = sc * c.cj + off + a;
            if (Y < 0 || Y >= g.H) continue;
            const float ly = (a + 0.5f) * inv_sc * fhalo;
            float L[NS], R[NS];
#pragma unroll
            for (int s = 0; s < NS; ++s) {
                L[s] = (1.f - ly) * t00[s] + ly * t10[s];
                R[s] = (1.f - ly) * t01[s] + ly * t11[s];
            }
            for (int bb = 0; bb < sc; ++bb) {
                const int t = __builtin_amdgcn_readlane(codes, a * sc + bb);
                if (t == -1) continue;
                if (t == -2) { bad = 1.f; continue; }
                const float lx = (bb + 0.5f) * inv_sc * fhalo;
                float z[NS], pr[NS];
#pragma unroll
                for (int s = 0; s < NS; ++s) z[s] = (lane + 64 * s) < g.C ? (1.f - lx) * L[s] + lx * R[s] : -INFINITY;
                const float lse = wave_softmax_bounded<NS>(z, mb, pr);
                const float wt = cw ? cw[t] : 1.f;
                nvalid += 1.f; wsum += wt;
#pragma unroll
                for (int s = 0; s < NS; ++s) {
                    aP[s] += pr[s];
                    if (lane + 64 * s == t) { aI[s] += pr[s]; aT[s] += 1.f; ce += wt * (lse - z[s]); }
                }
            }
        }
    }
    ce = wave_sum_all(ce);
    fwd_block_tail<NS>(aI, aP, aT, ce, wsum, nvalid, bad, lane, wave, g.C,
                       partial + ((int64_t)blockIdx.x * g.B + b) * (3 * g.C + 4));
}

template <typename T, int NS>
__global__ void __launch_bounds__(LS_THREADS) ce_dice_fwd_kernel(const T* __restrict__ logits, LossGeom g,
                                                                  const int64_t* __restrict__ target, int64_t ignore_index,
                                                                  const float* __restrict__ cw, float* __restrict__ partial) {
    const int lane = threadIdx.x & 63;
    const int wave = __builtin_amdgcn_readfirstlane(threadIdx.x >> 6);
    const int b = blockIdx.y;
    const int64_t npix = (int64_t)g.H * g.W;
    const int64_t nw = (int64_t)gridDim.x * 4;
    const int64_t per = (npix + nw - 1) / nw;
    const int64_t wid = (int64_t)blockIdx.x * 4 + wave;
    const int64_t p0 = wid * per, p1 = p0 + per < npix ? p0 + per : npix;
    const T* img = logits + (int64_t)b * g.h * g.w * g.ldl;
    const int64_t* tg = target + (int64_t)b * npix;
    float aI[NS], aP[NS], aT[NS];
#pragma unroll
    for (int s = 0; s < NS; ++s) { aI[s] = 0.f; aP[s] = 0.f; aT[s] = 0.f; }
    float ce = 0.f, wsum = 0.f, nvalid = 0.f, bad = 0.f;
    for (int64_t p = p0; p < p1; ++p) {
        const int64_t t = tg[p];
        if (t == ignore_index) continue;
        if (t < 0 || t >= g.C) { bad = 1.f; continue; }
        const int Y = (int)(p / g.W), X = (int)(p - (int64_t)Y * g.W);
        float z[NS], pr[NS];
        pixel_logits<T, NS>(img, g, Y, X, lane, z);
        const float lse = wave_softmax<NS>(z, pr);
        const float wt = cw ? cw[t] : 1.f;
        nvalid += 1.f; wsum += wt;
#pragma unroll
        for (int s = 0; s < NS; ++s) {
            aP[s] += pr[s];
            if (lane + 64 * s == (int)t) { aI[s] += pr[s]; aT[s] += 1.f; ce += wt * (lse - z[s]); }
        }
    }
    ce = wave_sum_all(ce);
    fwd_block_tail<NS>(aI, aP, aT, ce, wsum, nvalid, bad, lane, wave, g.C,
                       partial + ((int64_t)blockIdx.x * g.B + b) * (3 * g.C + 4));
}

__global__ void __launch_bounds__(256) ce_dice_loss_kernel(float* __restrict__ stats, int B, int C, int dice, float* __restrict__ loss) {
    __shared__ float red[256];
    __shared__ float tail[4];
    const int stride = 3 * C + 4;
    float dsum = 0.f;
    for (int i = threadIdx.x; i < B * C; i += 256) {
        const int b = i / C, c = i - b * C;
        const float* st = stats + (int64_t)b * stride;
        const float I = st[c], P = st[C + c], T = st[2 * C + c];
        float sets = P + T;
        if (sets == 0.f) sets = 2.f * I;
        dsum += (2.f * I + LS_EPS) / (sets + LS_EPS);
    }
    red[threadIdx.x] = dsum;
    if (threadIdx.x < 4) {
        float s = 0.f;
        for (int b = 0; b < B; ++b) s += stats[(int64_t)b * stride + 3 * C + threadIdx.x];
        tail[threadIdx.x] = s;
    }
    __syncthreads();
    for (int o = 128; o > 0; o >>= 1) {
        if (threadIdx.x < o) red[threadIdx.x] += red[threadIdx.x + o];
        __syncthreads();
    }
    if (threadIdx.x == 0) {
        float* st = stats + (int64_t)B * stride;
        st[0] = tail[0]; st[1] = tail[1]; st[2] = tail[2]; st[3] = tail[3];
        const float ce = tail[0] / tail[1];
        const float dl = dice ? 1.f - red[0] / (float)(B * C) : 0.f;
        loss[0] = ce + dl; loss[1] = ce; loss[2] = dl;
    }
}

template <int NS>
__device__ __forceinline__ void dice_coefs(const float* __restrict__ stats, int b, int B, int C, int dice, int lane,
                                           float (&gI)[NS], float (&gP)[NS]) {
    const float* st = stats + (int64_t)b * (3 * C + 4);
#pragma unroll
    for (int s = 0; s < NS; ++s) {
        const int c = lane + 64 * s;
        float a = 0.f, bb = 0.f;
        if (c < C && dice) {
            const float I = st[c], P = st[C + c], Tt = st[2 * C + c];
            const float sets = P + Tt;
            if (sets != 0.f) {
                const float nbc = 1.f / (float)(B * C);
                a = -nbc * 2.f / (sets + LS_EPS);
                bb = nbc * (2.f * I + LS_EPS) / ((sets + LS_EPS) * (sets + LS_EPS));
            }
        }
        gI[s] = a; gP[s] = bb;
    }
}
template <int NS>
__device__ __forceinline__ void pixel_grad(const float (&z)[NS], int t, int lane, const float (&gI)[NS], const float (&gP)[NS],
                                           float wce, float go, float (&dz)[NS], float mb = INFINITY) {
    float pr[NS], G[NS];
    if (mb == INFINITY) wave_softmax<NS>(z, pr); else wave_softmax_bounded<NS>(z, mb, pr);
    float dot = 0.f;
#pragma unroll
    for (int s = 0; s < NS; ++s) {
        G[s] = gP[s] + (lane + 64 * s == t ? gI[s] : 0.f);
        dot += G[s] * pr[s];
    }
    dot = wave_sum_all(dot);
#pragma unroll
    for (int s = 0; s < NS; ++s)
        dz[s] = go * (pr[s] * (G[s] - dot) + wce * (pr[s] - (lane + 64 * s == t ? 1.f : 0.f)));
}

template <typename T, int NS>
__global__ void __launch_bounds__(LS_THREADS) ce_dice_bwd_cells_kernel(const T* __restrict__ logits, LossGeom g, int sc,
                                                                        const int64_t* __restrict__ target, int64_t ignore_index,
                                                                        const float* __restrict__ cw, int dice,
                                                                        const float* __restrict__ stats,
                                                                        const float* __restrict__ grad_out, T* __restrict__ dlow,
                                                                        int64_t ldd, const int* __restrict__ run_if) {
    if (run_if && __hip_atomic_load(run_if, __ATOMIC_RELAXED, __HIP_MEMORY_SCOPE_AGENT) == 0) return;
    __shared__ float accum[LS_TILE * LS_TILE][64 * NS];
    const int lane = threadIdx.x & 63;
    const int wave = __builtin_amdgcn_readfirstlane(threadIdx.x >> 6);
    const int b = blockIdx.y;
    const int tiles_x = (g.w + LS_TILE - 1) / LS_TILE;
    const int ty0 = (blockIdx.x / tiles_x) * LS_TILE, tx0 = (blockIdx.x % tiles_x) * LS_TILE;
    const int halo = sc > 1 ? 1 : 0, off = sc >> 1;
    const float inv_sc = 1.f / (float)sc, fhalo = (float)halo;
    for (int i = threadIdx.x; i < LS_TILE * LS_TILE * 64 * NS; i += LS_THREADS) (&accum[0][0])[i] = 0.f;
    float gI[NS], gP[NS];
    dice_coefs<NS>(stats, b, g.B, g.C, dice, lane, gI, gP);
    const float go = grad_out ? grad_out[0] : 1.f;
    const float invW = 1.f / stats[(int64_t)g.B * (3 * g.C + 4) + 1];
    const T* img = logits + (int64_t)b * g.h * g.w * g.ldl;
    const int64_t* tg = target + (int64_t)b * g.H * g.W;
    __syncthreads();
    const int ncl = LS_TILE + halo;
    const int ncol = halo ? 4 : 1;
    for (int col = 0; col < ncol; ++col) {
        const int pj = col >> 1, pk = col & 1;
        const int nj = halo ? (ncl - pj + 1) / 2 : ncl, nk = halo ? (ncl - pk + 1) / 2 : ncl;
        for (int idx = wave; idx < nj * nk; idx += 4) {
            const int lj = halo ? 2 * (idx / nk) + pj : idx / nk, lk = halo ? 2 * (idx % nk) + pk : idx % nk;
            const int cj = ty0 - halo + lj, ck = tx0 - halo + lk;
// ... 1003 lines not shown
```

### segmentation_factory_amd/csrc/policy.h

```cpp
#pragma once

#define SEGF_POLICY_TABLE(X)                                                                                                             \
                                                                                                   \
    X(gemm_no_big, "SEGFAC_GEMM_NO_BIG", 0, "never take the 256 x 256-tile kernel (gemm_bf16_big_kernel): everything on the 128-tile one") \
    X(gemm_no_skinny, "SEGFAC_GEMM_NO_SKINNY", 0, "no streaming products for K, N <= 128 (gemm_skinny_kernel and its relatives)")        \
    X(gemm_no_skinny_rows, "SEGFAC_GEMM_NO_SKINNY_ROWS", 0, "the [tokens x 32] -> 768 projection on gemm_skinny_kernel instead of the whole-row form") \
    X(gemm_no_skinny_k, "SEGFAC_GEMM_NO_SKINNY_K", 0, "no K-split streaming product for 32- / 64-wide outputs (gemm_skinny_k_kernel)")  \
    X(gemm_no_dw_skinny, "SEGFAC_GEMM_NO_DW_SKINNY", 0, "small-output weight gradients on the tiled split-K kernel instead of gemm_dw_skinny_kernel") \
    X(gemm_no_narrow, "SEGFAC_GEMM_NO_NARROW", 0, "256-tile kernel: full 128 x 64 wave tiles also for outputs <= 160 wide (bit-identical results)") \
    X(gemm_no_deep, "SEGFAC_GEMM_NO_DEEP", 0, "256-tile forward: one K step of operand loads in flight instead of two")                  \
    X(gemm_no_deep128, "SEGFAC_GEMM_NO_DEEP128", 0, "128-tile kernel: one K step in flight instead of two")                              \
    X(gemm_no_fastload, "SEGFAC_GEMM_NO_FASTLOAD", 0, "guarded tile loads everywhere (no workgroup-uniform guard-free full-K-step loads)") \
    X(gemm_no_tr, "SEGFAC_GEMM_NO_TR", 0, "debugging: reduction-major fragments by scalar LDS reads instead of ds_read_b64_tr_b16; disables every kernel built on the transposed read") \
    X(gemm_no_pro, "SEGFAC_GEMM_NO_PRO", 0, "segf_gemm_pro_supported answers 0: BatchNorm + ReLU + Dropout2d are applied by their own pass") \
    X(gemm_no_fused_db, "SEGFAC_GEMM_NO_FUSED_DB", 0, "bias gradient as its own column-sum launch instead of riding on the weight-gradient product") \
    X(no_grouped_dw, "SEGFAC_NO_GROUPED_DW", 0, "segf_gemm_dw_db_grouped runs its members one by one")                                   \
    X(dw_no_xcd_slabs, "SEGFAC_DW_NO_XCD_SLABS", 0, "split-K weight gradients (128-tile kernel) in hardware workgroup order instead of one K slab per XCD")                \
    X(dw_no_shared_split, "SEGFAC_DW_NO_SHARED_SPLIT", 0, "grouped weight gradients keep their per-layer slice counts (also read by the host layer)") \
    X(no_wide_reduce, "SEGFAC_NO_WIDE_REDUCE", 0, "split-K partials of large outputs summed by the 16 x 16 form instead of whole rows")   \
    X(no_reduce4, "SEGFAC_NO_REDUCE4", 0, "split-K reduce: one output per thread instead of four (bitwise the same sums)")               \
    X(gemm_f32_no_mfma, "SEGFAC_GEMM_F32_NO_MFMA", 0, "fp32 storage (exact-parity mode, evaluate): products on the vector FMA kernel instead of the f32 matrix instruction") \
    X(gemm8_linear, "SEGFAC_GEMM8_LINEAR", 1, "0: plain nn.Linear products never take the eight-phase kernel (the 256 / 128 tile kernels as in r04)") \
    X(gemm8_linear_min_tiles, "SEGFAC_GEMM8_LINEAR_MIN_TILES", 128, "fewest 256 x 256 tiles for which a K >= 2048 nn.Linear product takes the eight-phase kernel (192 for shorter K)") \
    X(gemm8_linear_min_fill, "SEGFAC_GEMM8_LINEAR_MIN_FILL", 60, "smallest share (percent) of the launched 256 x 256 tiles that must be output for an nn.Linear product with ragged last tiles to take the eight-phase kernel") \
    X(gemm8_linear_min_k, "SEGFAC_GEMM8_LINEAR_MIN_K", 256, "shortest reduction for which an nn.Linear product takes the eight-phase kernel (its 12-load prologue and drain against K / 64 tiles)") \
    X(gemm8_dw, "SEGFAC_GEMM8_DW", 1, "0: nn.Linear weight gradients never take the eight-phase kernel below 65536 tokens (the grouped 128-tile kernel as in r04)") \
    X(gemm8_dw_min_gflop, "SEGFAC_GEMM8_DW_MIN_GFLOP", 100, "smallest nn.Linear weight gradient (GFLOP; both feature counts multiples of 256, >= 256 FLOP per operand byte) that takes the eight-phase kernel + a column-sum pass instead of the grouped 128-tile kernel") \
    X(gemm8_linear_min_gflop, "SEGFAC_GEMM8_LINEAR_MIN_GFLOP", 36, "smallest nn.Linear product (GFLOP, K >= 512; 100 for shorter K) that takes the eight-phase kernel") \
                                 \
    X(no_gemm8, "SEGFAC_NO_GEMM8", 0, "no eight-phase kernel at all (gemm8_kernel): the two-phase 256-tile kernel everywhere")           \
    X(no_gemm8t, "SEGFAC_NO_GEMM8T", 0, "no eight-phase kernel for weight gradients (reduction-major operands)")                         \
    X(conv_no_fwd_split, "SEGFAC_CONV_NO_FWD_SPLIT", 0, "3 x 3 forward / data gradient with few output tiles: no split over the (channel block, tap) walk") \
    X(g8_stagger, "SEGFAC_G8_STAGGER", -1, "eight-phase kernel: 1 = wave groups one barrier apart, 0 = lockstep, -1 = staggered for bf16 and the per-device choice (segf_gemm8_option) for fp8") \
    X(no_fp8, "SEGFAC_NO_FP8", 0, "segf_gemm_fp8_supported answers 0 (block-scaled 128-tile fp8 GEMM)")                                  \
    X(no_fp8_conv, "SEGFAC_NO_FP8_CONV", 0, "segf_conv3x3_fp8*_supported answer 0")                                                      \
    X(no_fp8_wgrad, "SEGFAC_NO_FP8_WGRAD", 0, "fp8 3 x 3 convolutions keep a bf16 weight gradient")                                      \
    X(no_fp8_linear, "SEGFAC_NO_FP8_LINEAR", 0, "segf_linear_fp8_supported answers 0")                                                   \
                                                                             \
    X(dilconv_no_cull, "SEGFAC_DILCONV_NO_CULL", 0, "dilated 3 x 3 convolution: all nine taps are walked, with zero loads where a tap leaves the image, instead of the live taps only") \
                                                                            \
    X(attn_no_mfma, "SEGFAC_ATTN_NO_MFMA", 0, "attention on the VALU reference kernels (attention.hip) also in bf16")                    \
    X(attn_f32_no_mfma, "SEGFAC_ATTN_F32_NO_MFMA", 0, "fp32 attention forward on the vector kernel (one query per lane) instead of the f32 matrix instruction") \
    X(attn64_prescale, "SEGFAC_ATTN64_PRESCALE", 0, "head dim 64, >= 128 keys: scale log2(e) rides on the Q fragments (bf16(q c), one more rounding per q element) and -max / -lse are the score accumulators' initial values, instead of one multiply-add per score: forward + query-side backward, +8 % / +2 % per kernel, attention error x 1.2 - 2.3") \
    X(attn64_dkv_rows, "SEGFAC_ATTN64_DKV_ROWS", 128, "head dim 64, >= 128 keys, key-side backward: query rows per staged Q / dO tile and barrier (128, 64 or 32: the same arithmetic, bit for bit)") \
    X(attn_no_fused_bwd, "SEGFAC_ATTN_NO_FUSED_BWD", 0, "head dim 32, <= 256 keys: query-side + key-side backward kernels instead of the one-kernel backward") \
    X(attn32_classic, "SEGFAC_ATTN32_CLASSIC", 0, "head dim 32 backward (one-kernel and key-side kernels): the round-2 score arithmetic (subtract, multiply, __expf; (dP - D) scale per score) instead of P = exp2(S c - lse log2(e)) with -D as the C operand of the dP products and the scale applied once to dK and dQ") \
                                                                                \
    X(dw_no_walk, "SEGFAC_DW_NO_WALK", 0, "depthwise 3 x 3: the round-1 strip kernels instead of the vertical-walk kernels")             \
    X(dw_walk_rows, "SEGFAC_DW_WALK_ROWS", 0, "depthwise 3 x 3 walk: rows per segment (0 = chosen from the map size)")                   \
    X(dw_no_small, "SEGFAC_DW_NO_SMALL", 0, "depthwise 3 x 3 backward of small maps: three passes instead of the one-launch LDS form")   \
    X(dw_small_always, "SEGFAC_DW_SMALL_ALWAYS", 0, "... the one-launch form beyond one round of workgroups as well")                    \
    X(ffn_bwd_fused, "SEGFAC_FFN_BWD_FUSED", 1, "Mix-FFN backward, fc2's data gradient formed inside pass A of the depthwise backward (segf_dwconv3x3_gelu_bwd_fc2_supported): 0 = never, 1 = from 131072 token rows on, 2 = wherever the shape has the kernel") \
                                                           \
    X(no_fuse_map, "SEGFAC_NO_FUSE_MAP", 0, "folded SegFormerHead map: streaming product + VALU upsample-add instead of fuse_map_kernel") \
    X(no_bwd248_mfma, "SEGFAC_NO_BWD248_MFMA", 0, "transposed 1/2-1/4-1/8 resizes on the VALU kernel instead of fuse_map_bwd_kernel")    \
    X(upadd_generic, "SEGFAC_UPADD_GENERIC", 0, "upsample-add: the generic per-source kernels also for the 2-4-8 pyramid")               \
    X(no_head_fused, "SEGFAC_NO_HEAD_FUSED", 0, "segf_bn_cls_bwd_supported answers 0: classifier data gradient and BatchNorm backward as separate passes") \
    X(no_head_fused_dw, "SEGFAC_NO_HEAD_FUSED_DW", 0, "the folded head's stage-1 weight gradient does not ride on pass 2 of the fused BatchNorm backward") \
                                                                                 \
    X(loss_no_band, "SEGFAC_LOSS_NO_BAND", 0, "CE / Dice forward and backward on the tile kernels instead of the band sweep")            \
    X(loss_no_band_fwd, "SEGFAC_LOSS_NO_BAND_FWD", 0, "... the forward only")                                                             \
    X(loss_band_rows, "SEGFAC_LOSS_BAND_ROWS", 0, "band sweep: rows per segment (0 = 16)")                                               \
    X(loss_no_mfma, "SEGFAC_LOSS_NO_MFMA", 0, "ratio-4 loss kernels on the VALU cells form (fp32 storage)")                              \
    X(loss_no_retry, "SEGFAC_LOSS_NO_RETRY", 0, "no exact per-pixel retry pass behind the flagged cells")                                \
    X(loss_no_lse, "SEGFAC_LOSS_NO_LSE", 0, "the backward recomputes the softmax normalisation instead of taking the forward's per-pixel log-sum") \
                                                                                                     \
    X(ln_linear_bwd_fused, "SEGFAC_LN_LINEAR_BWD_FUSED", 1, "Mix-FFN backward, fc1's data / weight / bias gradients formed inside the LayerNorm backward of norm2 (segf_layernorm_linear_bwd_supported): 0 = never, 1 = from 131072 token rows on, 2 = wherever the shape has the kernel") \
    X(ln_linear_fwd_fused, "SEGFAC_LN_LINEAR_FWD_FUSED", 1, "MiT stages 1 / 2: LayerNorm as the operand prologue of its thin Linear (norm2 -> fc1, norm1 -> q; segf_layernorm_linear_fwd_supported), the LayerNorm output neither stored nor saved, and norm1 -> q's backward in one pass where SEGFAC_LN_LINEAR_BWD_FUSED allows it too: 0 = never, 1 = from 131072 token rows on, 2 = wherever the shape has the kernel") \
                                                                                                 \
    X(no_wide_finalize, "SEGFAC_NO_WIDE_FINALIZE", 0, "column-reduction finalize: one output per thread instead of four (bitwise the same sums)") \
                                                                                 \
    X(no_ln_patch, "SEGFAC_NO_LN_PATCH", 0, "[host] MiT blocks: im2col / col2im around the spatial-reduction conv instead of the patch-major LayerNorm output") \
    X(no_scaled_ln_bwd, "SEGFAC_NO_SCALED_LN_BWD", 0, "[host] DropPath backward as its own scale_rows launch instead of riding on the LayerNorm backward") \
    X(no_deferred_dw, "SEGFAC_NO_DEFERRED_DW", 0, "[host] weight gradients issued layer by layer inside the captured step (no grouped launches)") \
    X(no_deferred_finalize, "SEGFAC_NO_DEFERRED_FINALIZE", 0, "[host] LayerNorm dgamma / dbeta finalizes issued one by one")              \
    X(no_head_fused_cw, "SEGFAC_NO_HEAD_FUSED_CW", 0, "[host] the classifier's weight gradient as its own product instead of riding on pass 1 of the fused BatchNorm backward") \
    X(no_bwd248, "SEGFAC_NO_BWD248", 0, "[host] folded head backward: three segf_bilinear_bwd launches instead of the one-pass segf_bilinear_bwd_248") \
    X(no_gelu_grn, "SEGFAC_NO_GELU_GRN", 0, "[host] ConvNeXtV2 blocks: GELU as its own pass in front of the GRN kernels")                \
    X(no_weight_shadow, "SEGFAC_NO_WEIGHT_SHADOW", 0, "[host] captured step: weights cast to bf16 per use instead of one cast of the flat buffer") \
    X(no_derived_weights, "SEGFAC_NO_DERIVED_WEIGHTS", 0, "[host] captured step: derived weight layouts built in front of each layer instead of one grouped launch")

struct SegfPolicy {
#define SEGF_POLICY_FIELD(field, env, def, doc) int field;
    SEGF_POLICY_TABLE(SEGF_POLICY_FIELD)
#undef SEGF_POLICY_FIELD
    int g8_stagger_fp8;
};

const SegfPolicy& segf_policy();
#define POL(field) (segf_policy().field)

struct SegfTrace {
    int on;
    int dry;
    int n;
    const char* names[256];
    const char* where[256];
};
SegfTrace& segf_trace();
void segf_trace_note(const char* kernel_text, const char* where);
```

### segmentation_factory_amd/functional.py

```python
import contextlib

import torch
from torch.autograd import Function

from . import hip


def _rowmajor(t):
    return t if t.stride(-1) == 1 else t.contiguous()


_SHADOW = None


class shadow_scope:
    def __init__(self, table):
        self.table = table

    def __enter__(self):
        global _SHADOW
        self.prev, _SHADOW = _SHADOW, self.table
        return self

    def __exit__(self, *exc):
# ... 1034 lines not shown
    @staticmethod
    def backward(ctx, dy):
        x, sc = ctx.saved_tensors
        gs = gslot(ctx, 1)
        dx, dscale = hip.colscale_bwd(_rowmajor(dy), x, sc, dscale=gs.view(-1) if gs is not None and gs.is_contiguous() else None)
        return dx, dscale.view(ctx.pshape)


def col_scale(x, scale):
    return ColScaleFn.apply(x, scale)


@direct_grads(1, 2)
class DWConvGeluFn(Function):

    @staticmethod
    def forward(ctx, x, weight, bias, B, H, W, apply_gelu):
        x = x if x.is_contiguous() else x.contiguous()
        Cc = x.shape[1]
        w9 = weight.detach().reshape(Cc, 9).contiguous()
        b = bias.detach().contiguous() if bias is not None else None
        y = hip.dwconv3x3_gelu_fwd(x, w9, b, B, H, W, Cc, apply_gelu)
        ctx.save_for_backward(x, w9, b)
        ctx.meta = (B, H, W, Cc, apply_gelu, weight.shape)
        return y

    @staticmethod
    def backward(ctx, dy):
        x, w9, b = ctx.saved_tensors
        B, H, W, Cc, apply_gelu, wshape = ctx.meta
        dy = dy if dy.is_contiguous() else dy.contiguous()
        gw, gb = gslot(ctx, 1), (gslot(ctx, 2) if b is not None else None)
        if _FIN_QUEUE is not None and _adjacent_slots(ctx, 1, 2) is not None:
            dx, item = hip.dwconv3x3_gelu_bwd(x, w9, b, dy, B, H, W, Cc, apply_gelu, dw_out=gw, db_out=gb, defer=True)
            _queue_finalizes(ctx, (item, (1, 2)))
            return dx, None, None, None, None, None, None
        dx, dw, db = hip.dwconv3x3_gelu_bwd(x, w9, b, dy, B, H, W, Cc, apply_gelu, dw_out=gw, db_out=gb)
        return dx, dw.view(wshape), (db if b is not None else None), None, None, None, None


def dwconv3x3_gelu(x, weight, bias, B, H, W, apply_gelu=True):
    return DWConvGeluFn.apply(x, weight, bias, B, H, W, apply_gelu)


@direct_grads(1, 2, 3, 4)
class DWConvGeluLinearFn(Function):

    @staticmethod
    def forward(ctx, x, weight2, bias2, weight, bias, B, H, W, residual, rscale):
        x = x if x.is_contiguous() else x.contiguous()
        M, Cc = x.shape
        N = weight2.shape[0]
        w9 = weight.detach().reshape(Cc, 9).contiguous()
        b = bias.detach().contiguous()
        g = hip.dwconv3x3_gelu_fwd(x, w9, b, B, H, W, Cc, True)
        w2 = _w(weight2.reshape(N, -1), x.dtype)
        y = hip.gemm(0, g, w2, M, N, Cc, bias=bias2.detach(), residual=residual, rscale=rscale, rows_per_group=H * W)
        ctx.save_for_backward(x, w9, b, g, w2, rscale)
        ctx.meta = (B, H, W, Cc, N, M, weight.shape, weight2.shape, residual is not None)
        return y

    @staticmethod
    def backward(ctx, dy):
        x, w9, b, g, w2, rscale = ctx.saved_tensors
        B, H, W, Cc, N, M, wshape, w2shape, has_res = ctx.meta
        dy = _rowmajor(dy)
        dys = _scaled_dy(dy, rscale, H * W) if rscale is not None else dy
        dw2, db2 = _linear_param_grads(ctx, dys, g, N, Cc, M, 1, 2, True, w2shape)
        gw, gb = gslot(ctx, 3), gslot(ctx, 4)
        dres = dy if (has_res and ctx.needs_input_grad[8]) else None
        if _FIN_QUEUE is not None and _adjacent_slots(ctx, 3, 4) is not None:
            dx, item = hip.dwconv3x3_gelu_bwd_fc2(x, w9, b, dys, w2, B, H, W, Cc, N, dw_out=gw, db_out=gb, defer=True)
            _queue_finalizes(ctx, (item, (3, 4)))
            return dx, dw2, db2, None, None, None, None, None, dres, None
        dx, dw, db = hip.dwconv3x3_gelu_bwd_fc2(x, w9, b, dys, w2, B, H, W, Cc, N, dw_out=gw, db_out=gb)
        return dx, dw2, db2, dw.view(wshape), db, None, None, None, dres, None


def dwconv3x3_gelu_linear_ok(x, weight2, bias2, weight, bias, B, H, W):
    if not (x.is_cuda and x.dtype == torch.bfloat16 and torch.is_grad_enabled() and x.requires_grad):
        return False
    if bias is None or bias2 is None or not all(p.requires_grad for p in (weight2, bias2, weight, bias)):
        return False
    return hip.dwconv3x3_gelu_bwd_fc2_supported(x.dtype, B, H, W, x.shape[1], weight2.shape[0])


def dwconv3x3_gelu_linear(x, weight2, bias2, weight, bias, B, H, W, residual=None, rscale=None):
    y = DWConvGeluLinearFn.apply(x, weight2, bias2, weight, bias, B, H, W, residual, rscale)
    if rscale is not None:
        y._segf_dp = (rscale, H * W)
    return y


def _bn_mean_rstd(x, training, pre_sums, running_mean, running_var, momentum, eps):
    if training and pre_sums is not None:
        return hip.bn_stats_from_sums(pre_sums, x.shape[0], running_mean, running_var, momentum, eps)
    if training:
        return hip.bn_stats(x, running_mean, running_var, momentum, eps)
    return running_mean.detach().clone(), torch.rsqrt(running_var.detach() + eps)


@direct_grads(1, 2)
class BatchNormActFn(Function):

    @staticmethod
    def forward(ctx, x, gamma, beta, running_mean, running_var, training, momentum, eps, act, chan_scale, rows_per_sample,
                pre_sums=None):
        x = x if x.is_contiguous() else x.contiguous()
        g, b = gamma.detach().contiguous(), beta.detach().contiguous()
        mean, rstd = _bn_mean_rstd(x, training, pre_sums, running_mean, running_var, momentum, eps)
        y = hip.bn_apply(x, mean, rstd, g, b, act, chan_scale, rows_per_sample or 1)
        ctx.save_for_backward(x, mean, rstd, g, b, chan_scale)
        ctx.meta = (act, rows_per_sample or 1, not training)
        return y

    @staticmethod
    def backward(ctx, dy):
        x, mean, rstd, g, b, chan_scale = ctx.saved_tensors
        act, rps, eval_mode = ctx.meta
        dy = dy if dy.is_contiguous() else dy.contiguous()
        dx, dg, db = hip.bn_bwd(x, dy, mean, rstd, g, b, act, chan_scale, rps, eval_mode)
        return dx, dg, db, None, None, None, None, None, None, None, None, None


def batch_norm_act(x, gamma, beta, running_mean, running_var, training, momentum=0.1, eps=1e-5, act=1, chan_scale=None,
                   rows_per_sample=None, pre_sums=None):
    return BatchNormActFn.apply(x, gamma, beta, running_mean, running_var, training, momentum, eps, act, chan_scale,
                                rows_per_sample, pre_sums)


@direct_grads(1, 2, 11, 12)
class BnActLinearFn(Function):

    @staticmethod
    def forward(ctx, x, gamma, beta, running_mean, running_var, training, momentum, eps, act, chan_scale, rps, weight, bias, Np,
                pre_sums, fold_slot=None):
        ctx.fold_slot = fold_slot
        x = x if x.is_contiguous() else x.contiguous()
        M, K = x.shape
        N = weight.shape[0]
        g, b = gamma.detach().contiguous(), beta.detach().contiguous()
        mean, rstd = _bn_mean_rstd(x, training, pre_sums, running_mean, running_var, momentum, eps)
        scale, shift = hip.bn_affine_table(mean, rstd, g, b, chan_scale, M // rps, K)
        w, bp = _padded_rows(weight, bias, N, Np, K, x.dtype, x.device)
        y = hip.gemm_pro(0, x, w, M, Np, K, scale, shift, rps, act, bias=bp)[:, :N]
        ctx.save_for_backward(x, mean, rstd, g, b, chan_scale, scale, shift, w)
        ctx.meta = (M, N, K, Np, act, rps, not training, bias is not None, weight.shape)
        return y

    @staticmethod
    def backward(ctx, dy):
        x, mean, rstd, g, b, chan_scale, scale, shift, w = ctx.saved_tensors
        M, N, K, Np, act, rps, eval_mode, has_bias, wshape = ctx.meta
        if dy.stride(-1) == 1 and dy.stride(0) == Np:
            dyp = dy.as_strided((M, Np), (Np, 1))
        else:
            dyp = hip.zeros((M, Np), x.dtype, x.device)
            hip.cast2d(_rowmajor(dy), dyp[:, :N])
        db = hip.colsum(dyp)[:N] if has_bias else None
        dw = None
        if hip.bn_cls_bwd_supported(x.dtype, M, K, Np, rps):
            slot = ctx.fold_slot
            x1 = slot.get('x1') if slot is not None else None
            ride_dg = x1 is not None and x1.shape[0] == M and hip.bn_cls_bwd_dw_supported(x.dtype, M, K, Np, rps, x1.shape[1])
            if act in (0, 1) and not hip.policy('no_head_fused_cw'):
                dx, dg, dbeta, dG, dwc = hip.bn_cls_bwd_full(dyp, w, x, mean, rstd, g, b, act, chan_scale, rps, eval_mode,
                                                             x1=x1 if ride_dg else None)
                dw = dwc[:N].view(wshape)
                if ride_dg:
                    slot['dG'] = dG
            elif ride_dg:
                dx, dg, dbeta, slot['dG'] = hip.bn_cls_bwd_dw(dyp, w, x, mean, rstd, g, b, act, chan_scale, rps, eval_mode, x1)
            else:
                dx, dg, dbeta = hip.bn_cls_bwd(dyp, w, x, mean, rstd, g, b, act, chan_scale, rps, eval_mode)
        else:
            da = hip.gemm(1, dyp, w, M, K, Np)
            dx, dg, dbeta = hip.bn_bwd(x, da, mean, rstd, g, b, act, chan_scale, rps, eval_mode)
        if dw is None:
            dw = hip.gemm_pro(2, dyp, x, Np, K, M, scale, shift, rps, act, split_k=_splitk(Np, K, M))[:N].view(wshape)
        return dx, dg, dbeta, None, None, None, None, None, None, None, None, dw, db, None, None, None


def bn_act_linear(x, gamma, beta, running_mean, running_var, training, momentum, eps, act, chan_scale, rows_per_sample, weight,
                  bias, pad_to=None, pre_sums=None):
    M, K = x.shape
    N = weight.shape[0]
    Np = pad_to if (pad_to and pad_to > N) else N
    rps = rows_per_sample or M
    if (x.dtype == torch.bfloat16 and act in (0, 1) and M % rps == 0 and hip.gemm_pro_supported(x.dtype, 0, M, Np, K, rps)
            and hip.gemm_pro_supported(x.dtype, 2, Np, K, M, rps)):
        return BnActLinearFn.apply(x, gamma, beta, running_mean, running_var, training, momentum, eps, act, chan_scale, rps,
                                   weight, bias, Np, pre_sums, getattr(x, '_segf_fold', None))
    y = batch_norm_act(x, gamma, beta, running_mean, running_var, training, momentum, eps, act, chan_scale, rows_per_sample,
                       pre_sums=pre_sums)
    return linear(y, weight, bias, pad_to=pad_to)


@direct_grads(5, 6, 7, 8, 9, 10, 11, 12)
class SegformerProjectConcatFn(Function):

    @staticmethod
    def forward(ctx, geoms, *args):
        feats, weights, biases = args[0:4], args[4:8], args[8:12]
        B = geoms[0][0]
        H1, W1 = geoms[0][1], geoms[0][2]
        E = weights[0].shape[0]
        dtype = feats[0].dtype
        M1 = B * H1 * W1
        cat = torch.empty((M1, 4 * E), dtype=dtype, device=feats[0].device)
        saved = []
        for i in range(4):
            f = _rowmajor(feats[i])
            w = _w(weights[i], dtype)
            _, h, wd = geoms[i]
            sl = cat[:, (3 - i) * E:(4 - i) * E]
            if i == 0:
                hip.gemm(0, f, w, M1, E, f.shape[1], out=sl, bias=biases[i].detach())
            else:
                t = hip.gemm(0, f, w, B * h * wd, E, f.shape[1], bias=biases[i].detach())
                hip.bilinear_fwd(t, B, h, wd, E, H1, W1, sl, align_corners=False)
            saved += [f, w]
        ctx.save_for_backward(*saved)
        ctx.meta = (geoms, E)
        return cat

    @staticmethod
    def backward(ctx, dcat):
        geoms, E = ctx.meta
        saved = ctx.saved_tensors
        dcat = _rowmajor(dcat)
        B, H1, W1 = geoms[0]
        dfs, dws, dbs = [], [], []
        for i in range(4):
            f, w = saved[2 * i], saved[2 * i + 1]
            _, h, wd = geoms[i]
            sl = dcat[:, (3 - i) * E:(4 - i) * E]
            dy = sl if i == 0 else hip.bilinear_bwd(sl, B, h, wd, E, H1, W1, align_corners=False)
            M, Ci = f.shape
            dfs.append(hip.gemm(1, dy, w, M, Ci, E) if ctx.needs_input_grad[1 + i] else None)
            dws.append(hip.gemm(2, dy, f, E, Ci, M, out_dtype=torch.float32, split_k=_splitk(E, Ci, M)))
            dbs.append(hip.colsum(dy))
        return (None, *dfs, *dws, *dbs)


def segformer_project_concat(feats, weights, biases, geoms):
    return SegformerProjectConcatFn.apply(tuple(geoms), *feats, *weights, *biases)


@direct_grads(5, 6, 7, 8, 9, 10, 11, 12, 13)
class SegformerFoldedFuseFn(Function):
# ... 624 lines not shown
```

### segmentation_factory_amd/hip.py

```python
import ctypes as C
import math
import os
import re

import torch

_HERE = os.path.dirname(os.path.abspath(__file__))
LIB_PATH = os.environ.get('SEGFAC_HIP_LIB') or os.path.join(_HERE, 'libsegfac_hip.so')
HEADER_PATH = os.path.normpath(os.path.join(_HERE, '..', 'include', 'segfac.h'))
F32, BF16 = 0, 1
ERR_SHAPE = -1
_lib = None

_i, _l, _f, _p = C.c_int, C.c_int64, C.c_float, C.c_void_p
_SCALAR = {'int': _i, 'int32_t': _i, 'int64_t': _l, 'float': _f}
_POINTEE = {'void', 'char', 'int', 'int32_t', 'int64_t', 'uint8_t', 'uint64_t', 'float'}


def _ctype(ctype, where, structs):
    t = re.sub(r'\bconst\b', ' ', ctype).replace('*', ' * ').split()
    if t and all(w == '*' for w in t[1:]):
        base, stars = t[0], len(t) - 1
        if stars == 0 and base in _SCALAR:
            return _SCALAR[base]
# ... 771 lines not shown
    y = torch.empty_like(x)
    _chk(lib().segf_bn_apply(dt_of(x), rows, Cc, _ptr(x), _ptr(mean), _ptr(rstd), _ptr(gamma), _ptr(beta), act,
                             _ptr(chan_scale), rows_per_sample, _ptr(y), _stream()), 'segf_bn_apply')
    return y


def bn_bwd(x, dy, mean, rstd, gamma, beta, act, chan_scale, rows_per_sample, eval_mode):
    rows, Cc = x.shape
    dx = torch.empty_like(x)
    dgamma = torch.empty(Cc, dtype=torch.float32, device=x.device)
    dbeta = torch.empty(Cc, dtype=torch.float32, device=x.device)
    ws = _f32(lib().segf_bn_ws(rows, Cc), x.device)
    _chk(lib().segf_bn_bwd(dt_of(x), rows, Cc, _ptr(x), _ptr(dy), _ptr(mean), _ptr(rstd), _ptr(gamma), _ptr(beta), act,
                           _ptr(chan_scale), rows_per_sample, int(eval_mode), _ptr(dx), _ptr(dgamma), _ptr(dbeta),
                           _ptr(ws), _stream()), 'segf_bn_bwd')
    return dx, dgamma, dbeta


def bn_cls_bwd_supported(dtype, M, Cc, K, rps):
    return dtype == torch.bfloat16 and bool(lib().segf_bn_cls_bwd_supported(BF16, M, Cc, K, rps))


def bn_cls_bwd(dy, w, x, mean, rstd, gamma, beta, act, chan_scale, rows_per_sample, eval_mode):
    _need_cuda(dy, w, x)
    M, Cc = x.shape
    K = w.shape[0]
    assert dy.shape[0] == M and dy.stride(1) == 1 and dy.stride(0) >= K and w.shape[1] == Cc and w.is_contiguous() and x.is_contiguous()
    dx = torch.empty_like(x)
    dgamma = torch.empty(Cc, dtype=torch.float32, device=x.device)
    dbeta = torch.empty(Cc, dtype=torch.float32, device=x.device)
    ws = _f32(lib().segf_bn_cls_bwd_ws(M, Cc, rows_per_sample), x.device)
    _chk(lib().segf_bn_cls_bwd(BF16, M, Cc, K, _ptr(dy), dy.stride(0), _ptr(w), w.stride(0), _ptr(x), _ptr(mean), _ptr(rstd),
                               _ptr(gamma), _ptr(beta), act, _ptr(chan_scale), rows_per_sample, int(eval_mode), _ptr(dx),
                               _ptr(dgamma), _ptr(dbeta), _ptr(ws), _stream()), 'segf_bn_cls_bwd')
    return dx, dgamma, dbeta


def bn_cls_bwd_dw_supported(dtype, M, Cc, K, rps, C1):
    return dtype == torch.bfloat16 and bool(lib().segf_bn_cls_bwd_dw_supported(BF16, M, Cc, K, rps, C1))


def bn_cls_bwd_dw(dy, w, x, mean, rstd, gamma, beta, act, chan_scale, rows_per_sample, eval_mode, x1):
    _need_cuda(dy, w, x, x1)
    M, Cc = x.shape
    K, C1 = w.shape[0], x1.shape[1]
    assert dy.shape[0] == M and dy.stride(1) == 1 and dy.stride(0) >= K and w.shape[1] == Cc and w.is_contiguous() and x.is_contiguous()
    assert x1.shape[0] == M and x1.stride(1) == 1 and x1.dtype == torch.bfloat16
    dx = torch.empty_like(x)
    dgamma = torch.empty(Cc, dtype=torch.float32, device=x.device)
    dbeta = torch.empty(Cc, dtype=torch.float32, device=x.device)
    dG = torch.empty((Cc, C1 + 8), dtype=torch.float32, device=x.device)
    ws = _f32(lib().segf_bn_cls_bwd_dw_ws(M, Cc, rows_per_sample), x.device)
    _chk(lib().segf_bn_cls_bwd_dw(BF16, M, Cc, K, _ptr(dy), dy.stride(0), _ptr(w), w.stride(0), _ptr(x), _ptr(mean), _ptr(rstd),
                                  _ptr(gamma), _ptr(beta), act, _ptr(chan_scale), rows_per_sample, int(eval_mode), _ptr(dx),
                                  _ptr(dgamma), _ptr(dbeta), _ptr(ws), _ptr(x1), x1.stride(0), C1, _ptr(dG), _stream()),
         'segf_bn_cls_bwd_dw')
    return dx, dgamma, dbeta, dG


def bn_cls_bwd_full(dy, w, x, mean, rstd, gamma, beta, act, chan_scale, rows_per_sample, eval_mode, x1=None, want_dwcls=True):
    _need_cuda(dy, w, x)
    M, Cc = x.shape
    K = w.shape[0]
    assert dy.shape[0] == M and dy.stride(1) == 1 and dy.stride(0) >= K and w.shape[1] == Cc and w.is_contiguous() and x.is_contiguous()
    assert act in (0, 1) or not want_dwcls
    dx = torch.empty_like(x)
    dgamma = torch.empty(Cc, dtype=torch.float32, device=x.device)
    dbeta = torch.empty(Cc, dtype=torch.float32, device=x.device)
    dG, C1 = None, 0
    if x1 is not None:
        assert x1.shape[0] == M and x1.stride(1) == 1 and x1.dtype == torch.bfloat16
        C1 = x1.shape[1]
        dG = torch.empty((Cc, C1 + 8), dtype=torch.float32, device=x.device)
    dwcls = torch.empty((K, Cc), dtype=torch.float32, device=x.device) if want_dwcls else None
    ws = _f32(lib().segf_bn_cls_bwd_full_ws(M, Cc, K, rows_per_sample), x.device)
    _chk(lib().segf_bn_cls_bwd_full(BF16, M, Cc, K, _ptr(dy), dy.stride(0), _ptr(w), w.stride(0), _ptr(x), _ptr(mean), _ptr(rstd),
                                    _ptr(gamma), _ptr(beta), act, _ptr(chan_scale), rows_per_sample, int(eval_mode), _ptr(dx),
                                    _ptr(dgamma), _ptr(dbeta), _ptr(ws), _ptr(x1) if x1 is not None else None,
                                    x1.stride(0) if x1 is not None else 0, C1, _ptr(dG) if dG is not None else None,
                                    _ptr(dwcls) if dwcls is not None else None, _stream()), 'segf_bn_cls_bwd_full')
    return dx, dgamma, dbeta, dG, dwcls


def grn_fwd(x, gamma, beta, B, rps, pre_gelu=False):
    Cc = x.shape[1]
    y = torch.empty_like(x)
    a = torch.empty((B, Cc), dtype=torch.float32, device=x.device)
    sq = torch.empty((B, Cc), dtype=torch.float32, device=x.device)
    ws = _f32(lib().segf_grn_ws(B, rps, Cc, 0), x.device)
    _chk(lib().segf_grn_fwd(dt_of(x), B, rps, Cc, _ptr(x), _ptr(gamma), _ptr(beta), _ptr(y), _ptr(a), _ptr(sq), _ptr(ws),
                            int(pre_gelu), _stream()), 'segf_grn_fwd')
    return y, sq


def grn_bwd(x, dy, gamma, sq, B, rps, pre_gelu=False):
    Cc = x.shape[1]
    dx = torch.empty_like(x)
    dgb = torch.empty((2, Cc), dtype=torch.float32, device=x.device)
    ws = _f32(lib().segf_grn_ws(B, rps, Cc, 1), x.device)
    _chk(lib().segf_grn_bwd(dt_of(x), B, rps, Cc, _ptr(x), _ptr(dy), _ptr(gamma), _ptr(sq), _ptr(dx), dgb[0].data_ptr(),
                            dgb[1].data_ptr(), _ptr(ws), int(pre_gelu), _stream()), 'segf_grn_bwd')
    return dx, dgb[0], dgb[1]


def attention_fwd(q, k, v, B, heads, N, Nkv, hd, scale):
    o = torch.empty((B * N, heads * hd), dtype=q.dtype, device=q.device)
    lse = torch.empty((B, heads, N), dtype=torch.float32, device=q.device)
    _chk(lib().segf_attention_fwd(dt_of(q), B, heads, N, Nkv, hd, _ptr(q), q.stride(0), _ptr(k), k.stride(0), _ptr(v),
                                  v.stride(0), scale, _ptr(o), o.stride(0), _ptr(lse), _stream()), 'segf_attention_fwd')
    return o, lse


def attention_bwd(q, k, v, o, d_o, lse, B, heads, N, Nkv, hd, scale, dk, dv):
    dq = torch.empty((B * N, heads * hd), dtype=q.dtype, device=q.device)
    ws = _f32(lib().segf_attention_bwd_ws(B, heads, N, Nkv, hd), q.device)
    _chk(lib().segf_attention_bwd(dt_of(q), B, heads, N, Nkv, hd, _ptr(q), q.stride(0), _ptr(k), k.stride(0), _ptr(v),
                                  v.stride(0), scale, _ptr(o), o.stride(0), _ptr(d_o), d_o.stride(0), _ptr(lse),
                                  _ptr(dq), dq.stride(0), _ptr(dk), dk.stride(0), _ptr(dv), dv.stride(0), _ptr(ws),
                                  _stream()), 'segf_attention_bwd')
    return dq


def _group_attention_check(t, B, H, W, heads, G, interval, lda):
    if G * G <= 64 and not lib().segf_group_attention_supported(dt_of(t), B, H, W, heads, 32, G, interval, int(lda)):
        raise RuntimeError(f'group attention: no kernel for a {H} x {W} map, batch {B}, {heads} heads of 32, groups of {G} x {G} '
                           f'({"LDA" if lda else "SDA"}, interval {interval}): sizes must be positive and B * H * W below 2^29')
    if G * G > 64:
        raise RuntimeError(f'group attention: no kernel for groups of {G} x {G} = {G * G} tokens ({"LDA" if lda else "SDA"}, interval '
                           f'{interval}) on a {H} x {W} map, batch {B}, {heads} heads of 32: a group holds at most 64 tokens '
                           f'(there is no fallback path)')


def group_attention_fwd(qkv, bias, B, H, W, heads, G, interval, lda, scale):
    _need_cuda(qkv, bias)
    _group_attention_check(qkv, B, H, W, heads, G, interval, lda)
    rows = B * H * W
    assert qkv.shape[0] == rows and qkv.stride(1) == 1 and bias.is_contiguous() and bias.dtype == torch.float32
    assert qkv.shape[1] >= 3 * heads * 32, f'qkv has {qkv.shape[1]} columns, {heads} heads of 32 need {3 * heads * 32}'
    assert tuple(bias.shape) == (heads, G * G, G * G), (tuple(bias.shape), heads, G)
    o = torch.empty((rows, heads * 32), dtype=qkv.dtype, device=qkv.device)
    lse = torch.empty((heads, rows), dtype=torch.float32, device=qkv.device)
    _chk(lib().segf_group_attention_fwd(dt_of(qkv), B, H, W, heads, 32, G, interval, int(lda), _ptr(qkv), qkv.stride(0), _ptr(bias),
                                        scale, _ptr(o), o.stride(0), _ptr(lse), _stream()), 'segf_group_attention_fwd')
    return o, lse


def group_attention_bwd(qkv, bias, d_o, lse, B, H, W, heads, G, interval, lda, scale):
    _need_cuda(qkv, bias, d_o)
    _group_attention_check(qkv, B, H, W, heads, G, interval, lda)
    assert qkv.shape[1] >= 3 * heads * 32 and d_o.shape[1] >= heads * 32 and d_o.stride(1) == 1
    dqkv = torch.empty((B * H * W, 3 * heads * 32), dtype=qkv.dtype, device=qkv.device)
    dbias = torch.empty((heads, G * G, G * G), dtype=torch.float32, device=qkv.device)
    ws = _f32(lib().segf_group_attention_bwd_ws(B, H, W, heads, 32, G, interval, int(lda)), qkv.device)
    _chk(lib().segf_group_attention_bwd(dt_of(qkv), B, H, W, heads, 32, G, interval, int(lda), _ptr(qkv), qkv.stride(0), _ptr(bias),
                                        scale, _ptr(d_o), d_o.stride(0), _ptr(lse), _ptr(dqkv), dqkv.stride(0), _ptr(dbias), _ptr(ws),
                                        _stream()), 'segf_group_attention_bwd')
    return dqkv, dbias


def _token_mixer_check(what, supported, B, HW, Cc, *ops):
    for t in ops:
        assert t.ndim == 2 and t.shape[0] == B * HW and t.shape[1] >= Cc and (t.stride(1) == 1 or t.shape[1] == 1), (what, tuple(t.shape))
    if not all(supported(dt_of(ops[0]), B, HW, Cc, ld) for ld in sorted({max(t.stride(0), Cc) if t.shape[0] == 1 else t.stride(0) for t in ops})):
        raise RuntimeError(f'{what}: no kernel for {B} x {HW} rows of {Cc} channels (leading dimensions {[t.stride(0) for t in ops]}): the '
                           f'channel count must be a multiple of 8 and at most 1024, B * HW below 2^29, rows 16-byte aligned '
                           f'(there is no fallback path)')
# ... 118 lines not shown
    if y is None:
        y = torch.empty((rows, cols), dtype=u.dtype, device=u.device)
    _metaformer_check('StarReLU', lib().segf_starrelu_supported, rows, cols, 8192, u, y)
    _chk(lib().segf_starrelu_fwd(dt_of(u), rows, cols, _ptr(u), _ld(u, cols), _ptr(_one_f32(s, 'StarReLU scale')),
                                 _ptr(_one_f32(b, 'StarReLU bias')), _ptr(y), _ld(y, cols), _stream()), 'segf_starrelu_fwd')
    return y


def starrelu_bwd(u, dy, s, du=None, ds=None, db=None):
    _need_cuda(u, dy, s)
    rows, cols = u.shape
    if du is None:
        du = torch.empty((rows, cols), dtype=u.dtype, device=u.device)
    _metaformer_check('StarReLU backward', lib().segf_starrelu_supported, rows, cols, 8192, u, dy, du)
    assert dy.shape[1] == cols
    if ds is None:
        ds = torch.empty(1, dtype=torch.float32, device=u.device)
    if db is None:
        db = torch.empty(1, dtype=torch.float32, device=u.device)
    ws = _f32(lib().segf_starrelu_bwd_ws(rows, cols), u.device)
    _chk(lib().segf_starrelu_bwd(dt_of(u), rows, cols, _ptr(u), _ld(u, cols), _ptr(dy), _ld(dy, cols), _ptr(_one_f32(s, 'StarReLU scale')),
                                 _ptr(du), _ld(du, cols), _ptr(_one_f32(ds, 'ds')), _ptr(_one_f32(db, 'db')), _ptr(ws), _stream()),
         'segf_starrelu_bwd')
    return du, ds, db


def colscale_fwd(x, scale, y=None):
    _need_cuda(x, scale)
    rows, Cc = x.shape[0], scale.numel()
    if y is None:
        y = torch.empty((rows, Cc), dtype=x.dtype, device=x.device)
    _metaformer_check('residual scale', lib().segf_colscale_supported, rows, Cc, 2048, x, y)
    assert scale.dtype == torch.float32 and scale.is_contiguous() and scale.data_ptr() % 16 == 0
    _chk(lib().segf_colscale_fwd(dt_of(x), rows, Cc, _ptr(x), _ld(x, Cc), _ptr(scale), _ptr(y), _ld(y, Cc), _stream()), 'segf_colscale_fwd')
    return y


def colscale_bwd(dy, x, scale, dx=None, dscale=None):
    _need_cuda(dy, x, scale)
    rows, Cc = x.shape[0], scale.numel()
    if dx is None:
        dx = torch.empty((rows, Cc), dtype=x.dtype, device=x.device)
    _metaformer_check('residual scale backward', lib().segf_colscale_supported, rows, Cc, 2048, dy, x, dx)
    assert scale.dtype == torch.float32 and scale.is_contiguous() and scale.data_ptr() % 16 == 0
    if dscale is None:
        dscale = torch.empty(Cc, dtype=torch.float32, device=x.device)
    assert dscale.dtype == torch.float32 and dscale.is_contiguous() and dscale.numel() == Cc
    ws = _f32(lib().segf_colscale_bwd_ws(rows, Cc), x.device)
    _chk(lib().segf_colscale_bwd(dt_of(x), rows, Cc, _ptr(dy), _ld(dy, Cc), _ptr(x), _ld(x, Cc), _ptr(scale), _ptr(dx), _ld(dx, Cc),
                                 _ptr(dscale), _ptr(ws), _stream()), 'segf_colscale_bwd')
    return dx, dscale


def dwconv3x3_gelu_fwd(x, w9, bias, B, H, W, Cc, apply_gelu=True):
    y = torch.empty_like(x)
    _chk(lib().segf_dwconv3x3_gelu_fwd(dt_of(x), B, H, W, Cc, _ptr(x), _ptr(w9), _ptr(bias), int(apply_gelu), _ptr(y),
                                       _stream()), 'segf_dwconv3x3_gelu_fwd')
    return y


def dwconv3x3_gelu_bwd(x, w9, bias, dy, B, H, W, Cc, apply_gelu=True, dw_out=None, db_out=None, defer=False):
    du = torch.empty_like(x)
    dx = torch.empty_like(x)
    if defer:
        assert dw_out.dtype == db_out.dtype == torch.float32 and dw_out.is_contiguous() and dw_out.numel() == 9 * Cc
        assert db_out.numel() == Cc and db_out.data_ptr() == dw_out.data_ptr() + 36 * Cc
        ws = _f32(lib().segf_dwconv3x3_bwd_ws(B, H, W, Cc), x.device)
        _chk(lib().segf_dwconv3x3_gelu_bwd(dt_of(x), B, H, W, Cc, _ptr(x), _ptr(w9), _ptr(bias), int(apply_gelu), _ptr(dy),
                                           _ptr(du), _ptr(dx), None, None, _ptr(ws), _stream()), 'segf_dwconv3x3_gelu_bwd')
        return dx, (ws, int(lib().segf_dwconv3x3_bwd_blocks(dt_of(x), B, H, W, Cc)), 10 * Cc, dw_out, Cc)
    dw = dw_out if dw_out is not None else torch.empty((Cc, 9), dtype=torch.float32, device=x.device)
    db = db_out if db_out is not None else torch.empty(Cc, dtype=torch.float32, device=x.device)
    assert dw.is_contiguous() and dw.numel() == Cc * 9 and db.is_contiguous() and db.numel() == Cc and dw.dtype == db.dtype == torch.float32
    ws = _f32(lib().segf_dwconv3x3_bwd_ws(B, H, W, Cc), x.device)
    _chk(lib().segf_dwconv3x3_gelu_bwd(dt_of(x), B, H, W, Cc, _ptr(x), _ptr(w9), _ptr(bias), int(apply_gelu), _ptr(dy),
                                       _ptr(du), _ptr(dx), _ptr(dw), _ptr(db), _ptr(ws), _stream()),
         'segf_dwconv3x3_gelu_bwd')
    return dx, dw, db


def dwconv3x3_gelu_bwd_fc2_supported(dtype, B, H, W, Cc, Cin):
    dt = BF16 if dtype == torch.bfloat16 else F32
    return bool(lib().segf_dwconv3x3_gelu_bwd_fc2_supported(dt, B, H, W, Cc, Cin))


def dwconv3x3_gelu_bwd_fc2(x, w9, bias, dys, w2, B, H, W, Cc, Cin, dw_out=None, db_out=None, defer=False, return_du=False):
    _need_cuda(x, dys, w2)
    assert x.dtype == dys.dtype == w2.dtype == torch.bfloat16 and x.is_contiguous() and w2.is_contiguous()
    assert dys.shape == (B * H * W, Cin) and dys.stride(1) == 1 and w2.shape == (Cin, Cc)
    du = torch.empty_like(x)
    dx = torch.empty_like(x)
    ws = _f32(lib().segf_dwconv3x3_bwd_ws(B, H, W, Cc), x.device)
    if defer:
        assert dw_out.dtype == db_out.dtype == torch.float32 and dw_out.is_contiguous() and dw_out.numel() == 9 * Cc
        assert db_out.numel() == Cc and db_out.data_ptr() == dw_out.data_ptr() + 36 * Cc
        blocks = int(lib().segf_dwconv3x3_bwd_blocks(dt_of(x), B, H, W, Cc))
        _chk(lib().segf_dwconv3x3_gelu_bwd_fc2(BF16, B, H, W, Cc, Cin, _ptr(x), _ptr(w9), _ptr(bias), _ptr(dys), dys.stride(0), _ptr(w2),
                                               _ptr(du), _ptr(dx), None, None, _ptr(ws), _stream()), 'segf_dwconv3x3_gelu_bwd_fc2')
        out = (dx, (ws, blocks, 10 * Cc, dw_out, Cc))
        return out + (du,) if return_du else out
    dw = dw_out if dw_out is not None else torch.empty((Cc, 9), dtype=torch.float32, device=x.device)
    db = db_out if db_out is not None else torch.empty(Cc, dtype=torch.float32, device=x.device)
    assert dw.is_contiguous() and dw.numel() == Cc * 9 and db.is_contiguous() and db.numel() == Cc and dw.dtype == db.dtype == torch.float32
    _chk(lib().segf_dwconv3x3_gelu_bwd_fc2(BF16, B, H, W, Cc, Cin, _ptr(x), _ptr(w9), _ptr(bias), _ptr(dys), dys.stride(0), _ptr(w2),
                                           _ptr(du), _ptr(dx), _ptr(dw), _ptr(db), _ptr(ws), _stream()), 'segf_dwconv3x3_gelu_bwd_fc2')
    return (dx, dw, db, du) if return_du else (dx, dw, db)


def dwconv7x7_fwd(x, wt49, bias, B, H, W, Cc):
    y = torch.empty_like(x)
    _chk(lib().segf_dwconv7x7_fwd(dt_of(x), B, H, W, Cc, _ptr(x), _ptr(wt49), _ptr(bias), _ptr(y), _stream()),
         'segf_dwconv7x7_fwd')
    return y


def dwconv7x7_bwd(x, wt49, dy, B, H, W, Cc, need_dx=True, need_db=True):
    dx = torch.empty_like(x) if need_dx else None
    dw = torch.empty((Cc, 49), dtype=torch.float32, device=x.device)
    db = torch.empty(Cc, dtype=torch.float32, device=x.device) if need_db else None
    ws = _f32(lib().segf_dwconv7x7_bwd_ws(B, H, W, Cc), x.device)
    _chk(lib().segf_dwconv7x7_bwd(dt_of(x), B, H, W, Cc, _ptr(x), _ptr(wt49), _ptr(dy), _ptr(dx), _ptr(dw), _ptr(db), _ptr(ws),
                                  _stream()), 'segf_dwconv7x7_bwd')
    return dx, dw, db


def conv3x3(mode, x, w, B, H, W, Cin, Cout, out=None, out_dtype=None, bias=None, split_k=1):
    _need_cuda(x, w)
    assert x.dtype == torch.bfloat16 and w.dtype == torch.bfloat16 and x.stride(-1) == 1 and w.stride(-1) == 1
    P = B * H * W
    shape = {0: (P, Cout), 1: (P, Cin), 2: (Cout, 9 * Cin)}[mode]
    if out is None:
        out = torch.empty(shape, dtype=out_dtype or (torch.float32 if mode == 2 else x.dtype), device=x.device)
    if mode != 2:
        split_k = int(lib().segf_conv3x3_fwd_splitk(mode, B, H, W, Cin, Cout)) if (bias is None and out.dtype == torch.bfloat16) else 1
    ws = _f32(split_k * shape[0] * shape[1], x.device) if split_k > 1 else None
    key = ('conv3x3', mode, P, Cin, Cout)
    _chk(_timed(key, lambda: lib().segf_conv3x3(mode, B, H, W, Cin, Cout, _ptr(x), x.stride(0), _ptr(w), w.stride(0), _ptr(out),
                                                dt_of(out), out.stride(0), _ptr(bias), split_k, _ptr(ws), _stream())),
         'segf_conv3x3')
    return out


def conv3x3_dil_live_taps(H, W, dilation):
    taps = (C.c_int * 9)()
    n = lib().segf_conv3x3_dil_live_taps(H, W, dilation, C.cast(taps, C.c_void_p))
    if n < 0:
        raise ValueError(f'conv3x3_dil_live_taps: bad geometry H={H} W={W} dilation={dilation}')
    return [int(taps[i]) for i in range(n)]


def conv3x3_dil_supported(dtype, mode, B, H, W, Cin, Cout, dilation):
    dt = BF16 if dtype == torch.bfloat16 else (F32 if dtype == torch.float32 else -1)
    return bool(lib().segf_conv3x3_dil_supported(dt, mode, B, H, W, Cin, Cout, dilation))


def pick_splitk_conv3x3_dil(B, H, W, Cin, Cout, dilation):
    return lib().segf_conv3x3_dil_pick_splitk(B, H, W, Cin, Cout, dilation)


def conv3x3_dil(mode, x, w, B, H, W, Cin, Cout, dilation, out=None):
    _need_cuda(x, w)
    assert x.dtype == w.dtype and x.stride(-1) == 1 and w.stride(-1) == 1
    P = B * H * W
    shape = {0: (P, Cout), 1: (P, Cin), 2: (Cout, 9 * Cin)}[mode]
    if out is None:
        out = torch.empty(shape, dtype=torch.float32 if mode == 2 else x.dtype, device=x.device)
# ... 398 lines not shown
```

Measured before the change: 5019 images/sec.

## Extend fused dwconv-fc2 backward to wide stages, ride classifier bias grad, unroll small kernels

Extends the fused depthwise-conv/GELU backward with fc2 data gradient to the 160- and 256-channel MiT stages. The fc2 weights for those stages are staged in LDS instead of registers, and the row-ring depth and unroll are adapted to the wider channel count. Separately, the classifier bias gradient is accumulated inside pass 1 of the fused BatchNorm/classifier backward, removing its own column-sum launch. The Bernoulli drop-path scale kernel and the Dice loss reduction are also unrolled, with cheaper row indexing and a batched tail sum. This adds LDS pressure and more kernel variants, and changes the reduction order of the bias gradient.

```diff
diff --git a/include/segfac.h b/include/segfac.h
--- a/include/segfac.h
+++ b/include/segfac.h
@@ -162,6 +162,12 @@
                          const float* mean, const float* rstd, const float* gamma, const float* beta, int act,
                          const float* chan_scale, int64_t rows_per_sample, int eval_mode, void* dx, float* dgamma, float* dbeta,
                          float* ws, const void* x1, int64_t ldx1, int C1, float* dG, float* dwcls, void* stream);
+int segf_bn_cls_bwd_full_db_supported(int dt, int64_t M, int C, int K, int64_t rows_per_sample);
+int64_t segf_bn_cls_bwd_full_db_ws(int64_t M, int C, int K, int64_t rows_per_sample);
+int segf_bn_cls_bwd_full_db(int dt, int64_t M, int C, int K, const void* dy, int64_t ldy, const void* w, int64_t ldw, const void* x,
+                            const float* mean, const float* rstd, const float* gamma, const float* beta, int act,
+                            const float* chan_scale, int64_t rows_per_sample, int eval_mode, void* dx, float* dgamma, float* dbeta,
+                            float* ws, const void* x1, int64_t ldx1, int C1, float* dG, float* dwcls, float* dbcls, void* stream);
 
 int64_t segf_grn_ws(int B, int64_t rows_per_sample, int C, int bwd);
 int segf_grn_fwd(int dt, int B, int64_t rows_per_sample, int C, const void* x, const float* gamma, const float* beta, void* y,
@@ -232,6 +238,7 @@
 int segf_dwconv3x3_gelu_bwd_fc2(int dt, int B, int H, int W, int C_hidden, int C_in, const void* f, const float* w9,
                                 const float* bias, const void* dys, int64_t ld_dys, const void* w2, void* du, void* dx,
                                 float* dw, float* db, float* ws, void* stream);
+int segf_dwconv3x3_gelu_bwd_fc2_lds_supported(int dt, int B, int H, int W, int C_hidden, int C_in);
 
 int segf_dwconv7x7_fwd(int dt, int B, int H, int W, int C, const void* x, const float* wt, const float* bias, void* y,
                        void* stream);
diff --git a/segmentation_factory_amd/csrc/conv.hip b/segmentation_factory_amd/csrc/conv.hip
--- a/segmentation_factory_amd/csrc/conv.hip
+++ b/segmentation_factory_amd/csrc/conv.hip
@@ -255,14 +255,18 @@
                                                                      int64_t ld_dys, const bf16_t* __restrict__ w2,
                                                                      bf16_t* __restrict__ y, int B, int H, int W, int C, int R, int nseg) {
     typedef bf16_t T;
+    constexpr bool WL = KS > 2;
+    constexpr int ND = KS > 5 ? 1 : (WL ? 2 : 3);
+    constexpr int JU = ND == 2 ? 6 : 3;
     const int lane = threadIdx.x & 63;
     const int n = lane & 15, g = lane >> 4;
     const int nslab = C / 64;
     const int nrun = (W + 15) / 16;
     const int units = B * nseg * nrun;
     const int wv = __builtin_amdgcn_readfirstlane((int)(xcd_block() * 4 + (threadIdx.x >> 6)));
-    const int ustep = (int)((gridDim.x * 4) / nslab);
-    const int cbase = (wv % nslab) * 64;
+    const int ustep = WL ? (int)(gridDim.x / nslab) * 4 : (int)((gridDim.x * 4) / nslab);
+    const int cbase = (WL ? (wv >> 2) % nslab : wv % nslab) * 64;
+    const int u0 = WL ? ((wv >> 2) / nslab) * 4 + (wv & 3) : wv / nslab;
     const int c0 = cbase + 4 * n;
     f32x2_t wk[9][2], bs[2];
 #pragma unroll
@@ -271,20 +275,36 @@
         for (int kk = 0; kk < 9; ++kk) wk[kk][jj] = f32x2_t{w[(c0 + 2 * jj) * 9 + kk], w[(c0 + 2 * jj + 1) * 9 + kk]};
         bs[jj] = bias ? f32x2_t{bias[c0 + 2 * jj], bias[c0 + 2 * jj + 1]} : f32x2_t{0.f, 0.f};
     }
-    dwf_bf16x8 Bf[4][KS];
-#pragma unroll
-    for (int s = 0; s < KS; ++s) {
-        dwf_s16x8 t[4];
-#pragma unroll
-        for (int e = 0; e < 8; ++e) {
-            const uint2 q = *reinterpret_cast<const uint2*>(w2 + (int64_t)(32 * s + 8 * g + e) * C + c0);
-            t[0][e] = (short)(q.x & 0xffffu); t[1][e] = (short)(q.x >> 16); t[2][e] = (short)(q.y & 0xffffu); t[3][e] = (short)(q.y >> 16);
-        }
-#pragma unroll
-        for (int j = 0; j < 4; ++j) Bf[j][s] = __builtin_bit_cast(dwf_bf16x8, t[j]);
-    }
-    const int steps = (R + 2 + 2) / 3;
-    for (int u = wv / nslab; u < units; u += ustep) {
+    dwf_bf16x8 Bf[4][WL ? 1 : KS];
+    __shared__ dwf_u32x4 w2s[WL ? 4 * KS * 64 : 1];
+    if constexpr (!WL) {
+#pragma unroll
+        for (int s = 0; s < KS; ++s) {
+            dwf_s16x8 t[4];
+#pragma unroll
+            for (int e = 0; e < 8; ++e) {
+                const uint2 q = *reinterpret_cast<const uint2*>(w2 + (int64_t)(32 * s + 8 * g + e) * C + c0);
+                t[0][e] = (short)(q.x & 0xffffu); t[1][e] = (short)(q.x >> 16); t[2][e] = (short)(q.y & 0xffffu); t[3][e] = (short)(q.y >> 16);
+            }
+#pragma unroll
+            for (int j = 0; j < 4; ++j) Bf[j][s] = __builtin_bit_cast(dwf_bf16x8, t[j]);
+        }
+    } else {
+        for (int p = threadIdx.x; p < KS * 64; p += 256) {
+            const int s = p >> 6, l = p & 63;
+            dwf_s16x8 t[4];
+#pragma unroll
+            for (int e = 0; e < 8; ++e) {
+                const uint2 q = *reinterpret_cast<const uint2*>(w2 + (int64_t)(32 * s + 8 * (l >> 4) + e) * C + cbase + 4 * (l & 15));
+                t[0][e] = (short)(q.x & 0xffffu); t[1][e] = (short)(q.x >> 16); t[2][e] = (short)(q.y & 0xffffu); t[3][e] = (short)(q.y >> 16);
+            }
+#pragma unroll
+            for (int j = 0; j < 4; ++j) w2s[(j * KS + s) * 64 + l] = __builtin_bit_cast(dwf_u32x4, t[j]);
+        }
+        __syncthreads();
+    }
+    const int steps = (R + 2 + JU - 1) / JU;
+    for (int u = u0; u < units; u += ustep) {
         const int run = u % nrun;
         const int t = u / nrun;
         const int seg = t % nseg;
@@ -309,7 +329,7 @@
 #pragma unroll
             for (int p = 0; p < DW_PIX; ++p) { acc[a][p][0] = bs[0]; acc[a][p][1] = bs[1]; }
         Raw4<T> rawb[3][DW_PIX + 2];
-        dwf_u32x4 dysb[3][KS];
+        dwf_u32x4 dysb[ND][KS];
         auto load_row = [&](int yin, Raw4<T> (&dst)[DW_PIX + 2]) {
             const int yc = yin < 0 ? 0 : (yin >= H ? H - 1 : yin);
             const T* row = xb + (int64_t)yc * W * C;
@@ -324,18 +344,19 @@
         };
         load_row(ya - 1, rawb[0]);
         load_row(ya, rawb[1]);
-        load_grow(ya - 2, dysb[0]); load_grow(ya - 1, dysb[1]);
+        if constexpr (ND > 1) load_grow(ya - 2, dysb[0]);
+        if constexpr (ND > 2) load_grow(ya - 1, dysb[1]);
         int yin = ya - 1;
         for (int st = 0; st < steps; ++st) {
 #pragma unroll
-            for (int j = 0; j < 3; ++j, ++yin) {
+            for (int j = 0; j < JU; ++j, ++yin) {
                 f32x2_t (&P)[DW_PIX][2] = acc[j % 3];
                 f32x2_t (&Cc)[DW_PIX][2] = acc[(j + 1) % 3];
                 f32x2_t (&N)[DW_PIX][2] = acc[(j + 2) % 3];
                 Raw4<T> (&curc)[DW_PIX + 2] = rawb[j % 3];
-                dwf_u32x4 (&gcurc)[KS] = dysb[j % 3];
+                dwf_u32x4 (&gcurc)[KS] = dysb[j % ND];
                 load_row(yin + 2, rawb[(j + 2) % 3]);
-                load_grow(yin + 1, dysb[(j + 2) % 3]);
+                load_grow(yin + ND - 2, dysb[(j + ND - 1) % ND]);
                 const bool vy = yin >= 0 && yin < H && yin <= yb;
 #pragma unroll
                 for (int cx = 0; cx < DW_PIX + 2; ++cx) {
@@ -361,8 +382,12 @@
                     for (int jm = 0; jm < 4; ++jm) {
                         dgf[jm] = dwf_f32x4{0.f, 0.f, 0.f, 0.f};
 #pragma unroll
-                        for (int s = 0; s < KS; ++s)
-                            dgf[jm] = __builtin_amdgcn_mfma_f32_16x16x32_bf16(__builtin_bit_cast(dwf_bf16x8, gcurc[s]), Bf[jm][s], dgf[jm], 0, 0, 0);
+                        for (int s = 0; s < KS; ++s) {
+                            dwf_bf16x8 bfr;
+                            if constexpr (WL) bfr = __builtin_bit_cast(dwf_bf16x8, w2s[(jm * KS + s) * 64 + lane]);
+                            else bfr = Bf[jm][s];
+                            dgf[jm] = __builtin_amdgcn_mfma_f32_16x16x32_bf16(__builtin_bit_cast(dwf_bf16x8, gcurc[s]), bfr, dgf[jm], 0, 0, 0);
+                        }
                     }
                     T* orow = yo_b + (int64_t)yo * W * C;
 #pragma unroll
@@ -845,17 +870,26 @@
 }
 
 #define DW_FC2_MIN_ROWS 131072
-static inline bool dw_fc2_shape_ok(int dt, int B, int H, int W, int C, int Cin) {
-    return dt == SEGF_BF16 && B > 0 && H > 0 && W > 0 && (Cin == 32 || Cin == 64) && C > 0 && C % 64 == 0 &&
+static inline bool dw_fc2_lds_cin(int Cin) { return Cin == 160 || Cin == 256; }
+static inline bool dw_fc2_shape_ok(int dt, int B, int H, int W, int C, int Cin, bool lds = false) {
+    return dt == SEGF_BF16 && B > 0 && H > 0 && W > 0 && (lds ? dw_fc2_lds_cin(Cin) : (Cin == 32 || Cin == 64)) && C > 0 && C % 64 == 0 &&
            (int64_t)B * H * W < (1ll << 31);
 }
-extern "C" int segf_dwconv3x3_gelu_bwd_fc2_supported(int dt, int B, int H, int W, int C_hidden, int C_in) {
-    if (!dw_fc2_shape_ok(dt, B, H, W, C_hidden, C_in)) return 0;
+static int dw_fc2_supported(int dt, int B, int H, int W, int C_hidden, int C_in, bool lds, int64_t min_rows) {
+    if (!dw_fc2_shape_ok(dt, B, H, W, C_hidden, C_in, lds)) return 0;
     if (!dw_use_walk() || dw_small_nch(dt, B, H, W, C_hidden)) return 0;
     const int pol = POL(ffn_bwd_fused);
     if (pol <= 0) return 0;
     if (pol >= 2) return 1;
-    return (int64_t)B * H * W >= DW_FC2_MIN_ROWS;
+    return (int64_t)B * H * W >= min_rows;
+}
+extern "C" int segf_dwconv3x3_gelu_bwd_fc2_supported(int dt, int B, int H, int W, int C_hidden, int C_in) {
+    return dw_fc2_supported(dt, B, H, W, C_hidden, C_in, false, DW_FC2_MIN_ROWS);
+}
+#define DW_FC2_LDS_MIN_ROWS_160 16384
+#define DW_FC2_LDS_MIN_ROWS_256 32768
+extern "C" int segf_dwconv3x3_gelu_bwd_fc2_lds_supported(int dt, int B, int H, int W, int C_hidden, int C_in) {
+    return dw_fc2_supported(dt, B, H, W, C_hidden, C_in, true, C_in == 160 ? DW_FC2_LDS_MIN_ROWS_160 : DW_FC2_LDS_MIN_ROWS_256);
 }
 extern "C" int segf_dwconv3x3_gelu_bwd_fc2(int dt, int B, int H, int W, int C_hidden, int C_in, const void* f, const float* w9,
                                            const float* bias, const void* dys, int64_t ld_dys, const void* w2, void* du, void* dx,
@@ -863,7 +897,7 @@
     if (B <= 0 || H <= 0 || W <= 0) return 0;
     const int C = C_hidden;
     if (dt != SEGF_BF16) return SEGF_ERR_DTYPE;
-    if (!dw_fc2_shape_ok(dt, B, H, W, C, C_in) || !dw_use_walk() || dw_small_nch(dt, B, H, W, C)) return SEGF_ERR_SHAPE;
+    if (!dw_fc2_shape_ok(dt, B, H, W, C, C_in, dw_fc2_lds_cin(C_in)) || !dw_use_walk() || dw_small_nch(dt, B, H, W, C)) return SEGF_ERR_SHAPE;
     if (((uintptr_t)f % 16) || ((uintptr_t)dys % 16) || ((uintptr_t)w2 % 16) || ((uintptr_t)du % 16) || ((uintptr_t)dx % 16) ||
         ld_dys < C_in || ld_dys % 8 != 0)
         return SEGF_ERR_SHAPE;
@@ -878,7 +912,18 @@
         int64_t blocks = (waves + 3) / 4;
         if (blocks > 32768) blocks = 32768;
         blocks = (blocks + nslab - 1) / nslab * nslab;
-        if (C_in == 32)
+        if (dw_fc2_lds_cin(C_in)) {
+            const int64_t units = (int64_t)B * q.nseg * ((W + 15) / 16);
+            int64_t groups = (units + 3) / 4;
+            if (groups * nslab > 32768) groups = 32768 / nslab;
+            blocks = groups * nslab;
+            if (C_in == 160)
+                hipLaunchKernelGGL((dwconv3x3_walk_fc2_kernel<5>), dim3((unsigned)blocks), dim3(256), 0, st, (const T*)f, w9, bias, (const T*)dys,
+                                   ld_dys, (const T*)w2, (T*)du, B, H, W, C, q.R, q.nseg);
+            else
+                hipLaunchKernelGGL((dwconv3x3_walk_fc2_kernel<8>), dim3((unsigned)blocks), dim3(256), 0, st, (const T*)f, w9, bias, (const T*)dys,
+                                   ld_dys, (const T*)w2, (T*)du, B, H, W, C, q.R, q.nseg);
+        } else if (C_in == 32)
             hipLaunchKernelGGL((dwconv3x3_walk_fc2_kernel<1>), dim3((unsigned)blocks), dim3(256), 0, st, (const T*)f, w9, bias, (const T*)dys,
                                ld_dys, (const T*)w2, (T*)du, B, H, W, C, q.R, q.nseg);
         else
diff --git a/segmentation_factory_amd/csrc/elementwise.hip b/segmentation_factory_amd/csrc/elementwise.hip
--- a/segmentation_factory_amd/csrc/elementwise.hip
+++ b/segmentation_factory_amd/csrc/elementwise.hip
@@ -409,12 +409,30 @@
 __global__ void bernoulli_scale_kernel(uint64_t* __restrict__ state, const float* __restrict__ kp, int64_t n, int64_t row_len,
                                        float* __restrict__ out) {
     const uint64_t seed = state[0], ctr = state[1];
-    for (int64_t i = (int64_t)blockIdx.x * blockDim.x + threadIdx.x; i < n; i += (int64_t)gridDim.x * blockDim.x) {
-        const uint64_t r = splitmix64(splitmix64(seed ^ (ctr * 0xD1B54A32D192ED03ull)) + (uint64_t)i);
+    const uint64_t base = splitmix64(seed ^ (ctr * 0xD1B54A32D192ED03ull));
+    constexpr uint32_t BS_U = 8;
+    const uint32_t nn = (uint32_t)n, rl = row_len < n ? (uint32_t)row_len : nn;
+    const uint32_t step = gridDim.x * blockDim.x;
+    const uint32_t srow = step / rl, srem = step - srow * rl;
+    uint32_t i = blockIdx.x * blockDim.x + threadIdx.x;
+    uint32_t row = i / rl, rem = i - row * rl;
+    auto advance = [&]() {
+        row += srow; rem += srem;
+        if (rem >= rl) { rem -= rl; ++row; }
+    };
+    auto scale = [&](uint32_t e, float k) {
+        const uint64_t r = splitmix64(base + (uint64_t)e);
         const float u = (float)(r >> 40) * (1.f / 16777216.f);
-        const float k = kp[i / row_len];
-        out[i] = u < k ? 1.f / k : 0.f;
-    }
+        return u < k ? 1.f / k : 0.f;
+    };
+    for (; (uint64_t)i + (uint64_t)(BS_U - 1) * step < nn; i += BS_U * step) {
+        float k[BS_U];
+#pragma unroll
+        for (uint32_t j = 0; j < BS_U; ++j) { k[j] = kp[row]; advance(); }
+#pragma unroll
+        for (uint32_t j = 0; j < BS_U; ++j) out[i + j * step] = scale(i + j * step, k[j]);
+    }
+    for (; i < nn; i += step) { out[i] = scale(i, kp[row]); advance(); }
     __syncthreads();
     if (gridDim.x == 1 && threadIdx.x == 0) state[1] = ctr + 1;
 }
diff --git a/segmentation_factory_amd/csrc/head_fused.hip b/segmentation_factory_amd/csrc/head_fused.hip
--- a/segmentation_factory_amd/csrc/head_fused.hip
+++ b/segmentation_factory_amd/csrc/head_fused.hip
@@ -17,6 +17,7 @@
     const bf16_t* x1; int64_t ldx1;
     float* dwpart;
     float* cwpart;
+    float* dbpart;
 };
 #define DW_C1 32
 #define DW_LD 40
@@ -45,7 +46,7 @@
 #ifndef HF_U
 #define HF_U 4
 #endif
-template <int PASS, int KS, bool DW = false, bool CW = false>
+template <int PASS, int KS, bool DW = false, bool CW = false, bool DB = false>
 __global__ void __launch_bounds__(64 * HF_WAVES, HF_OCC) bn_cls_bwd_kernel(HeadFusedArgs a) {
     constexpr int NT = 2;
     constexpr int TOK = 16 * HF_U;
@@ -63,6 +64,8 @@
     static_assert(!DW || (PASS == 2 && HF_WAVES == 8 && TOK == 64), "the riding weight gradient belongs to pass 2");
     static_assert(!CW || (PASS == 1 && TOK % 32 == 0), "the classifier's weight gradient rides on pass 1");
     __shared__ __attribute__((aligned(16))) bf16_t at[CW ? TOK : 1][XRS];
+    static_assert(!DB || (PASS == 1 && HF_WAVES == 8 && TOK == 64), "the classifier's bias gradient rides on pass 1");
+    __shared__ __attribute__((aligned(16))) float dbs[DB ? HF_WAVES : 1][DB ? 32 * KS : 4];
     hf_f32x4 accc[CW ? 2 * KS : 1][CW ? 2 : 1];
 #pragma unroll
     for (int i = 0; i < (CW ? 2 * KS : 1); ++i)
@@ -191,11 +194,39 @@
     for (int i = 0; i < (DW ? 2 : 1); ++i)
 #pragma unroll
         for (int j = 0; j < (DW ? 3 : 1); ++j) accw[i][j] = hf_f32x4{0.f, 0.f, 0.f, 0.f};
+    const bool db_lane = DB && 4 * lane < 32 * KS;
+    if (DB) *reinterpret_cast<float4*>(&dbs[wave][db_lane ? 4 * lane : 0]) = make_float4(0.f, 0.f, 0.f, 0.f);
+    int db_turn = slice;
     if (gbeg < gend) { fetch_tile(gbeg); fetch_x(gbeg); fetch_x1(gbeg); stash_tile(0); stash_x(0); stash_x1(0, gbeg); }
     __syncthreads();
     int bufi = 0;
     for (int gp = gbeg; gp < gend; gp += HF_U) {
         const bool more = gp + HF_U < gend;
+        if (DB) {
+            const bool mine = db_turn == 0;
+            db_turn = mine ? ny - 1 : db_turn - 1;
+            if (mine && db_lane && gp + (wave >> 1) < gend) {
+                float4 h8 = make_float4(0.f, 0.f, 0.f, 0.f);
+#pragma unroll 1
+                for (int t0 = 0; t0 < 8; t0 += 4) {
+                    uint2 q[4];
+#pragma unroll
+                    for (int t = 0; t < 4; ++t) q[t] = *reinterpret_cast<const uint2*>(&tile[bufi][8 * wave + t0 + t][4 * lane]);
+                    h8.x += (__uint_as_float(q[0].x << 16) + __uint_as_float(q[1].x << 16)) +
+                            (__uint_as_float(q[2].x << 16) + __uint_as_float(q[3].x << 16));
+                    h8.y += (__uint_as_float(q[0].x & 0xffff0000u) + __uint_as_float(q[1].x & 0xffff0000u)) +
+                            (__uint_as_float(q[2].x & 0xffff0000u) + __uint_as_float(q[3].x & 0xffff0000u));
+                    h8.z += (__uint_as_float(q[0].y << 16) + __uint_as_float(q[1].y << 16)) +
+                            (__uint_as_float(q[2].y << 16) + __uint_as_float(q[3].y << 16));
+                    h8.w += (__uint_as_float(q[0].y & 0xffff0000u) + __uint_as_float(q[1].y & 0xffff0000u)) +
+                            (__uint_as_float(q[2].y & 0xffff0000u) + __uint_as_float(q[3].y & 0xffff0000u));
+                }
+                float4 sv = *reinterpret_cast<const float4*>(&dbs[wave][4 * lane]);
+                sv.x += h8.x; sv.y += h8.y; sv.z += h8.z; sv.w += h8.w;
+                *reinterpret_cast<float4*>(&dbs[wave][4 * lane]) = sv;
+            }
+            __builtin_amdgcn_sched_barrier(0);
+        }
         if (more) { fetch_tile(gp + HF_U); fetch_x(gp + HF_U); fetch_x1(gp + HF_U); }
         constexpr int UNR = CW ? 1 : HF_U;
 #pragma unroll UNR
@@ -312,6 +343,14 @@
 #pragma unroll
                 for (int r = 0; r < 4; ++r) dst[(int64_t)(16 * ct + 4 * g + r) * a.C + 16 * ft] = accc[ct][ft][r];
     }
+    if (DB) {
+        __syncthreads();
+        if ((int)threadIdx.x < 32 * KS) {
+            const int t = (int)threadIdx.x;
+            const float sv = ((dbs[0][t] + dbs[1][t]) + (dbs[2][t] + dbs[3][t])) + ((dbs[4][t] + dbs[5][t]) + (dbs[6][t] + dbs[7][t]));
+            a.dbpart[((int64_t)blk * ny + slice) * (32 * KS) + t] = sv;
+        }
+    }
     if (PASS == 1) {
         float* dst = a.partial + (int64_t)blk * 2 * a.C + f0;
 #pragma unroll
@@ -329,6 +368,20 @@
     if (c >= C) return;
     dbeta[c] = sums[c];
     dgamma[c] = sums[C + c];
+}
+
+__global__ void __launch_bounds__(256) hf_db_finalize_kernel(const float* __restrict__ part, int nparts, int K, float* __restrict__ out) {
+    __shared__ double red[256];
+    const int k = blockIdx.x;
+    double s = 0.0;
+    for (int b = threadIdx.x; b < nparts; b += 256) s += (double)part[(int64_t)b * K + k];
+    red[threadIdx.x] = s;
+    __syncthreads();
+    for (int o = 128; o > 0; o >>= 1) {
+        if ((int)threadIdx.x < o) red[threadIdx.x] += red[threadIdx.x + o];
+        __syncthreads();
+    }
+    if (threadIdx.x == 0) out[k] = (float)red[0];
 }
 
 static int hf_chunks(int B, int groups_per_sample, int ny, bool cw = false) {
@@ -370,7 +423,37 @@
 static int bn_cls_bwd_impl(int dt, int64_t M, int C, int K, const void* dy, int64_t ldy, const void* w, int64_t ldw, const void* x,
                            const float* mean, const float* rstd, const float* gamma, const float* beta, int act,
                            const float* chan_scale, int64_t rows_per_sample, int eval_mode, void* dx, float* dgamma,
-                           float* dbeta, float* ws, const void* x1, int64_t ldx1, float* dG, void* stream, float* dwcls = nullptr);
+                           float* dbeta, float* ws, const void* x1, int64_t ldx1, float* dG, void* stream, float* dwcls = nullptr,
+                           float* dbcls = nullptr);
+
+#define HF_DB_MIN_ROWS 131072
+extern "C" int segf_bn_cls_bwd_full_db_supported(int dt, int64_t M, int C, int K, int64_t rows_per_sample) {
+    if (!segf_bn_cls_bwd_supported(dt, M, C, K, rows_per_sample)) return 0;
+    const int pol = POL(head_db_ride);
+    if (pol <= 0) return 0;
+    if (pol >= 2) return 1;
+    return M >= HF_DB_MIN_ROWS;
+}
+extern "C" int64_t segf_bn_cls_bwd_full_db_ws(int64_t M, int C, int K, int64_t rows_per_sample) {
+    const int B = (int)(M / rows_per_sample);
+    const int ny = C / (32 * HF_WAVES);
+    const int64_t nb = (int64_t)B * hf_chunks(B, (int)(rows_per_sample / 16), ny, true);
+    const int64_t used = nb * 2 * C + 2 * C + nb * C * DW_LD + nb * (int64_t)K * C + nb * ny * K;
+    const int64_t full = segf_bn_cls_bwd_full_ws(M, C, K, rows_per_sample);
+    return used > full ? used : full;
+}
+extern "C" int segf_bn_cls_bwd_full_db(int dt, int64_t M, int C, int K, const void* dy, int64_t ldy, const void* w, int64_t ldw,
+                                       const void* x, const float* mean, const float* rstd, const float* gamma, const float* beta, int act,
+                                       const float* chan_scale, int64_t rows_per_sample, int eval_mode, void* dx, float* dgamma,
+                                       float* dbeta, float* ws, const void* x1, int64_t ldx1, int C1, float* dG, float* dwcls,
+                                       float* dbcls, void* stream) {
+    if (!segf_bn_cls_bwd_full_db_supported(dt, M, C, K, rows_per_sample) || !dwcls || !dbcls) return SEGF_ERR_SHAPE;
+    if (x1 && (!segf_bn_cls_bwd_dw_supported(dt, M, C, K, rows_per_sample, C1) || !dG || ldx1 < C1 || ldx1 % 8 || ((uintptr_t)x1 % 16)))
+        return SEGF_ERR_SHAPE;
+    if (K > 192 || act > 1) return SEGF_ERR_SHAPE;
+    return bn_cls_bwd_impl(dt, M, C, K, dy, ldy, w, ldw, x, mean, rstd, gamma, beta, act, chan_scale, rows_per_sample, eval_mode, dx,
+                           dgamma, dbeta, ws, x1, ldx1, x1 ? dG : nullptr, stream, dwcls, dbcls);
+}
 
 extern "C" int segf_bn_cls_bwd_full(int dt, int64_t M, int C, int K, const void* dy, int64_t ldy, const void* w, int64_t ldw,
                                     const void* x, const float* mean, const float* rstd, const float* gamma, const float* beta, int act,
@@ -404,7 +487,7 @@
 static int bn_cls_bwd_impl(int dt, int64_t M, int C, int K, const void* dy, int64_t ldy, const void* w, int64_t ldw, const void* x,
                            const float* mean, const float* rstd, const float* gamma, const float* beta, int act,
                            const float* chan_scale, int64_t rows_per_sample, int eval_mode, void* dx, float* dgamma,
-                           float* dbeta, float* ws, const void* x1, int64_t ldx1, float* dG, void* stream, float* dwcls) {
+                           float* dbeta, float* ws, const void* x1, int64_t ldx1, float* dG, void* stream, float* dwcls, float* dbcls) {
     if (!segf_bn_cls_bwd_supported(dt, M, C, K, rows_per_sample) || ldy < K || ldw < C || act < 0 || act > 2) return SEGF_ERR_SHAPE;
     if (((uintptr_t)dy | (uintptr_t)x | (uintptr_t)dx) % 16 || (ldy % 8)) return SEGF_ERR_SHAPE;
     if (!ws) return SEGF_ERR_WORKSPACE;
@@ -415,8 +498,9 @@
     float* sums = ws + (int64_t)nblk * 2 * C;
     float* dwpart = sums + 2 * C;
     float* cwpart = dwpart + (int64_t)nblk * C * DW_LD;
+    float* dbpart = cwpart + (int64_t)nblk * K * C;
     HeadFusedArgs a{(const bf16_t*)dy, ldy, (const bf16_t*)w, ldw, (const bf16_t*)x, mean, rstd, gamma, beta, chan_scale, sums,
-                    (bf16_t*)dx, ws, M, C, rows_per_sample, gps, chunks, act, eval_mode, (const bf16_t*)x1, ldx1, dwpart, cwpart};
+                    (bf16_t*)dx, ws, M, C, rows_per_sample, gps, chunks, act, eval_mode, (const bf16_t*)x1, ldx1, dwpart, cwpart, dbpart};
     const dim3 grid((unsigned)(nblk * ny));
 #define HF_LAUNCH(PASS)                                                                                                  \
     do {                                                                                                                 \
@@ -429,7 +513,20 @@
         default: hipLaunchKernelGGL((bn_cls_bwd_kernel<PASS, 6>), grid, dim3(64 * HF_WAVES), 0, st, a); break;                     \
         }                                                                                                                \
     } while (0)
-    if (dwcls) {
+    if (dwcls && dbcls) {
+        switch (K / 32) {
+        case 1: hipLaunchKernelGGL((bn_cls_bwd_kernel<1, 1, false, true, true>), grid, dim3(64 * HF_WAVES), 0, st, a); break;
+        case 2: hipLaunchKernelGGL((bn_cls_bwd_kernel<1, 2, false, true, true>), grid, dim3(64 * HF_WAVES), 0, st, a); break;
+        case 3: hipLaunchKernelGGL((bn_cls_bwd_kernel<1, 3, false, true, true>), grid, dim3(64 * HF_WAVES), 0, st, a); break;
+        case 4: hipLaunchKernelGGL((bn_cls_bwd_kernel<1, 4, false, true, true>), grid, dim3(64 * HF_WAVES), 0, st, a); break;
+        case 5: hipLaunchKernelGGL((bn_cls_bwd_kernel<1, 5, false, true, true>), grid, dim3(64 * HF_WAVES), 0, st, a); break;
+        default: hipLaunchKernelGGL((bn_cls_bwd_kernel<1, 6, false, true, true>), grid, dim3(64 * HF_WAVES), 0, st, a); break;
+        }
+        SEGF_CHECK_LAUNCH();
+        colreduce_finalize_launch(cwpart, nblk, (int64_t)K * C, dwcls, st);
+        SEGF_CHECK_LAUNCH();
+        hipLaunchKernelGGL(hf_db_finalize_kernel, dim3(K), dim3(256), 0, st, dbpart, nblk * ny, K, dbcls);
+    } else if (dwcls) {
         switch (K / 32) {
         case 1: hipLaunchKernelGGL((bn_cls_bwd_kernel<1, 1, false, true>), grid, dim3(64 * HF_WAVES), 0, st, a); break;
         case 2: hipLaunchKernelGGL((bn_cls_bwd_kernel<1, 2, false, true>), grid, dim3(64 * HF_WAVES), 0, st, a); break;
diff --git a/segmentation_factory_amd/csrc/loss.hip b/segmentation_factory_amd/csrc/loss.hip
--- a/segmentation_factory_amd/csrc/loss.hip
+++ b/segmentation_factory_amd/csrc/loss.hip
@@ -394,24 +394,50 @@
 }
 
 __global__ void __launch_bounds__(256) ce_dice_loss_kernel(float* __restrict__ stats, int B, int C, int dice, float* __restrict__ loss) {
+    constexpr int LD_U = 8;
     __shared__ float red[256];
     __shared__ float tail[4];
+    __shared__ float tch[256 * 4];
     const int stride = 3 * C + 4;
+    const int n = B * C;
     float dsum = 0.f;
-    for (int i = threadIdx.x; i < B * C; i += 256) {
+    auto term = [](float I, float P, float T) {
+        float sets = P + T;
+        if (sets == 0.f) sets = 2.f * I;
+        return (2.f * I + LS_EPS) / (sets + LS_EPS);
+    };
+    int i = threadIdx.x;
+    for (; i + (LD_U - 1) * 256 < n; i += LD_U * 256) {
+        float I[LD_U], P[LD_U], T[LD_U];
+#pragma unroll
+        for (int j = 0; j < LD_U; ++j) {
+            const int e = i + j * 256, b = e / C, c = e - b * C;
+            const float* st = stats + (int64_t)b * stride;
+            I[j] = st[c]; P[j] = st[C + c]; T[j] = st[2 * C + c];
+        }
+#pragma unroll
+        for (int j = 0; j < LD_U; ++j) dsum += term(I[j], P[j], T[j]);
+    }
+    for (; i < n; i += 256) {
         const int b = i / C, c = i - b * C;
         const float* st = stats + (int64_t)b * stride;
-        const float I = st[c], P = st[C + c], T = st[2 * C + c];
-        float sets = P + T;
-        if (sets == 0.f) sets = 2.f * I;
-        dsum += (2.f * I + LS_EPS) / (sets + LS_EPS);
+        dsum += term(st[c], st[C + c], st[2 * C + c]);
     }
     red[threadIdx.x] = dsum;
-    if (threadIdx.x < 4) {
-        float s = 0.f;
-        for (int b = 0; b < B; ++b) s += stats[(int64_t)b * stride + 3 * C + threadIdx.x];
-        tail[threadIdx.x] = s;
-    }
+    float s = 0.f;
+    for (int b0 = 0; b0 < B; b0 += 256) {
+        const int nb = B - b0 < 256 ? B - b0 : 256;
+        if (b0) __syncthreads();
+#pragma unroll
+        for (int j = 0; j < 4; ++j) {
+            const int e = threadIdx.x + j * 256, b = e >> 2;
+            if (b < nb) tch[e] = stats[(int64_t)(b0 + b) * stride + 3 * C + (e & 3)];
+        }
+        __syncthreads();
+        if (threadIdx.x < 4)
+            for (int b = 0; b < nb; ++b) s += tch[b * 4 + threadIdx.x];
+    }
+    if (threadIdx.x < 4) tail[threadIdx.x] = s;
     __syncthreads();
     for (int o = 128; o > 0; o >>= 1) {
         if (threadIdx.x < o) red[threadIdx.x] += red[threadIdx.x + o];
diff --git a/segmentation_factory_amd/csrc/policy.h b/segmentation_factory_amd/csrc/policy.h
--- a/segmentation_factory_amd/csrc/policy.h
+++ b/segmentation_factory_amd/csrc/policy.h
@@ -57,7 +57,8 @@
     X(upadd_generic, "SEGFAC_UPADD_GENERIC", 0, "upsample-add: the generic per-source kernels also for the 2-4-8 pyramid")               \
     X(no_head_fused, "SEGFAC_NO_HEAD_FUSED", 0, "segf_bn_cls_bwd_supported answers 0: classifier data gradient and BatchNorm backward as separate passes") \
     X(no_head_fused_dw, "SEGFAC_NO_HEAD_FUSED_DW", 0, "the folded head's stage-1 weight gradient does not ride on pass 2 of the fused BatchNorm backward") \
-                                                                                 \
+    X(head_db_ride, "SEGFAC_HEAD_DB_RIDE", 1, "the classifier's bias gradient rides on pass 1 of the fused BatchNorm backward instead of a column-sum launch of its own (segf_bn_cls_bwd_full_db_supported): 0 = never, 1 = from 131072 token rows on, 2 = wherever the shape has the kernel") \
+                                                                                \
     X(loss_no_band, "SEGFAC_LOSS_NO_BAND", 0, "CE / Dice forward and backward on the tile kernels instead of the band sweep")            \
     X(loss_no_band_fwd, "SEGFAC_LOSS_NO_BAND_FWD", 0, "... the forward only")                                                             \
     X(loss_band_rows, "SEGFAC_LOSS_BAND_ROWS", 0, "band sweep: rows per segment (0 = 16)")                                               \
diff --git a/segmentation_factory_amd/functional.py b/segmentation_factory_amd/functional.py
--- a/segmentation_factory_amd/functional.py
+++ b/segmentation_factory_amd/functional.py
@@ -1140,7 +1140,8 @@
         return False
     if bias is None or bias2 is None or not all(p.requires_grad for p in (weight2, bias2, weight, bias)):
         return False
-    return hip.dwconv3x3_gelu_bwd_fc2_supported(x.dtype, B, H, W, x.shape[1], weight2.shape[0])
+    return (hip.dwconv3x3_gelu_bwd_fc2_supported(x.dtype, B, H, W, x.shape[1], weight2.shape[0])
+            or hip.dwconv3x3_gelu_bwd_fc2_lds_supported(x.dtype, B, H, W, x.shape[1], weight2.shape[0]))
 
 
 def dwconv3x3_gelu_linear(x, weight2, bias2, weight, bias, B, H, W, residual=None, rscale=None):
@@ -1215,15 +1216,22 @@
         else:
             dyp = hip.zeros((M, Np), x.dtype, x.device)
             hip.cast2d(_rowmajor(dy), dyp[:, :N])
-        db = hip.colsum(dyp)[:N] if has_bias else None
+        ride_db = (has_bias and act in (0, 1) and not hip.policy('no_head_fused_cw')
+                   and hip.bn_cls_bwd_full_db_supported(x.dtype, M, K, Np, rps))
+        db = hip.colsum(dyp)[:N] if has_bias and not ride_db else None
         dw = None
         if hip.bn_cls_bwd_supported(x.dtype, M, K, Np, rps):
             slot = ctx.fold_slot
             x1 = slot.get('x1') if slot is not None else None
             ride_dg = x1 is not None and x1.shape[0] == M and hip.bn_cls_bwd_dw_supported(x.dtype, M, K, Np, rps, x1.shape[1])
             if act in (0, 1) and not hip.policy('no_head_fused_cw'):
-                dx, dg, dbeta, dG, dwc = hip.bn_cls_bwd_full(dyp, w, x, mean, rstd, g, b, act, chan_scale, rps, eval_mode,
-                                                             x1=x1 if ride_dg else None)
+                if ride_db:
+                    dx, dg, dbeta, dG, dwc, dbc = hip.bn_cls_bwd_full_db(dyp, w, x, mean, rstd, g, b, act, chan_scale, rps, eval_mode,
+                                                                         x1=x1 if ride_dg else None)
+                    db = dbc[:N]
+                else:
+                    dx, dg, dbeta, dG, dwc = hip.bn_cls_bwd_full(dyp, w, x, mean, rstd, g, b, act, chan_scale, rps, eval_mode,
+                                                                 x1=x1 if ride_dg else None)
                 dw = dwc[:N].view(wshape)
                 if ride_dg:
                     slot['dG'] = dG
diff --git a/segmentation_factory_amd/hip.py b/segmentation_factory_amd/hip.py
--- a/segmentation_factory_amd/hip.py
+++ b/segmentation_factory_amd/hip.py
@@ -877,6 +877,35 @@
     return dx, dgamma, dbeta, dG, dwcls
 
 
+def bn_cls_bwd_full_db_supported(dtype, M, Cc, K, rps):
+    return dtype == torch.bfloat16 and bool(lib().segf_bn_cls_bwd_full_db_supported(BF16, M, Cc, K, rps))
+
+
+def bn_cls_bwd_full_db(dy, w, x, mean, rstd, gamma, beta, act, chan_scale, rows_per_sample, eval_mode, x1=None):
+    _need_cuda(dy, w, x)
+    M, Cc = x.shape
+    K = w.shape[0]
+    assert dy.shape[0] == M and dy.stride(1) == 1 and dy.stride(0) >= K and w.shape[1] == Cc and w.is_contiguous() and x.is_contiguous()
+    assert act in (0, 1)
+    dx = torch.empty_like(x)
+    dgamma = torch.empty(Cc, dtype=torch.float32, device=x.device)
+    dbeta = torch.empty(Cc, dtype=torch.float32, device=x.device)
+    dG, C1 = None, 0
+    if x1 is not None:
+        assert x1.shape[0] == M and x1.stride(1) == 1 and x1.dtype == torch.bfloat16
+        C1 = x1.shape[1]
+        dG = torch.empty((Cc, C1 + 8), dtype=torch.float32, device=x.device)
+    dwcls = torch.empty((K, Cc), dtype=torch.float32, device=x.device)
+    dbcls = torch.empty(K, dtype=torch.float32, device=x.device)
+    ws = _f32(lib().segf_bn_cls_bwd_full_db_ws(M, Cc, K, rows_per_sample), x.device)
+    _chk(lib().segf_bn_cls_bwd_full_db(BF16, M, Cc, K, _ptr(dy), dy.stride(0), _ptr(w), w.stride(0), _ptr(x), _ptr(mean), _ptr(rstd),
+                                       _ptr(gamma), _ptr(beta), act, _ptr(chan_scale), rows_per_sample, int(eval_mode), _ptr(dx),
+                                       _ptr(dgamma), _ptr(dbeta), _ptr(ws), _ptr(x1) if x1 is not None else None,
+                                       x1.stride(0) if x1 is not None else 0, C1, _ptr(dG) if dG is not None else None,
+                                       _ptr(dwcls), _ptr(dbcls), _stream()), 'segf_bn_cls_bwd_full_db')
+    return dx, dgamma, dbeta, dG, dwcls, dbcls
+
+
 def grn_fwd(x, gamma, beta, B, rps, pre_gelu=False):
     Cc = x.shape[1]
     y = torch.empty_like(x)
@@ -1161,6 +1190,11 @@
 def dwconv3x3_gelu_bwd_fc2_supported(dtype, B, H, W, Cc, Cin):
     dt = BF16 if dtype == torch.bfloat16 else F32
     return bool(lib().segf_dwconv3x3_gelu_bwd_fc2_supported(dt, B, H, W, Cc, Cin))
+
+
+def dwconv3x3_gelu_bwd_fc2_lds_supported(dtype, B, H, W, Cc, Cin):
+    dt = BF16 if dtype == torch.bfloat16 else F32
+    return bool(lib().segf_dwconv3x3_gelu_bwd_fc2_lds_supported(dt, B, H, W, Cc, Cin))
 
 
 def dwconv3x3_gelu_bwd_fc2(x, w9, bias, dys, w2, B, H, W, Cc, Cin, dw_out=None, db_out=None, defer=False, return_du=False):
```

After: 5085 images/sec, median of 6. +1.3%, better.
